# Tom-Ryder/VIforSDEs

Measured on AMD Instinct MI355X. Metric: sampled-paths/sec + ELBO-iters/sec (value = global_batch * ELBO-iters/s), higher is better.
Workload: dtype f32 (GRU/ELBO kernels) + bf16-autocast encoder

## Files before the change

include/vsde_hip.h:

```cpp
#ifndef VSDE_HIP_H
#define VSDE_HIP_H

#include <stddef.h>
#include <stdint.h>

#ifdef __cplusplus
extern "C" {
#endif

#define VSDE_ABI_VERSION 1

#define VSDE_E_BADARG (-1)
#define VSDE_E_LAYERS (-2)
#define VSDE_E_HIDDEN (-3)
#define VSDE_E_WORKSPACE (-4)
#define VSDE_E_STATE (-5)

#define VSDE_MAX_LAYERS 4
#define VSDE_MAX_HIDDEN 1024
#define VSDE_MAX_STATE 32

#define VSDE_CTX_F32 0
#define VSDE_CTX_BF16 1

// ... 59 lines not shown

int vsde_elbo_path_terms_bwd(int B, int T, int S, const float *z, const float *x,
                             const float *means, const float *chol, const float *drift,
                             const float *diffusion, const uint8_t *positive_mask_host,
                             double time_step, const float *g_sde, const float *g_gen,
                             const float *g_jac, float *g_z, float *g_x, float *g_means,
                             float *g_chol, float *g_drift, float *g_diffusion, void *stream);

int vsde_ln_modulate_fwd(int dtype, const void *x, const void *scale, const void *shift, void *y, float *mean,
                         float *rstd, int64_t B, int N, int C, double eps, int64_t mod_pitch, void *stream);
size_t vsde_colsum_workspace_bytes(int64_t B, int C);
int vsde_ln_modulate_bwd(int dtype, const void *x, const void *scale, const void *dy, const float *mean,
                         const float *rstd, const void *dres, void *dx, void *dscale, void *dshift, int64_t B, int N, int C,
                         int64_t mod_pitch, void *workspace, size_t workspace_bytes, void *stream);
int vsde_residual_ln_fwd(int dtype, const void *x, const void *y, const void *gate, const void *scale, const void *shift,
                         void *xnew, void *h, float *mean, float *rstd, int64_t B, int N, int C, double eps, int64_t mod_pitch,
                         void *stream);
int vsde_residual_ln_bwd(int dtype, const void *xnew, const void *y, const void *gate, const void *scale, const void *dh,
                         const void *dxnew, const float *mean, const float *rstd, void *dx, void *dy, void *dgate,
                         void *dscale, void *dshift, int64_t B, int N, int C, int64_t mod_pitch, void *workspace,
                         size_t workspace_bytes, void *stream);
int vsde_gated_residual_fwd(int dtype, const void *x, const void *y, const void *gate, void *out, int64_t B, int N, int C,
                            int64_t mod_pitch, void *stream);
int vsde_gated_residual_bwd(int dtype, const void *y, const void *gate, const void *dout, void *dy, void *dgate, int64_t B,
                            int N, int C, int64_t mod_pitch, void *workspace, size_t workspace_bytes, void *stream);
int vsde_swiglu_fwd(int dtype, const void *u, void *out, int64_t M, int H2, void *stream);
int vsde_swiglu_bwd(int dtype, const void *u, const void *dout, void *du, int64_t M, int H2, void *stream);
int vsde_gate_merge_fwd(int dtype, const void *attn, const void *glog, void *out, int64_t B, int N, int heads, int d,
                        int token_major, int64_t glog_stride, void *stream);
int vsde_gate_merge_bwd(int dtype, const void *attn, const void *glog, const void *dout, void *dattn, void *dglog, int64_t B,
                        int N, int heads, int d, int token_major, int64_t glog_stride, void *stream);
int vsde_qk_norm_rope_fwd(int dtype, const void *qkv, const float *cosT, const float *sinT, const float *wq, const float *wk,
                          const void *v0, const float *lam, void *q, void *k, void *v, int64_t B, int N, int heads, int d,
                          double eps, int token_major, int64_t row_stride, void *stream);
int64_t vsde_qk_norm_rope_bwd_partials(int64_t B, int N, int heads, int d);
int vsde_qk_norm_rope_bwd(int dtype, const void *qkv, const float *cosT, const float *sinT, const float *wq, const float *wk,
                          const void *v0, const float *lam, const void *dq, const void *dk, const void *dv, void *dqkv,
                          void *dv0, float *dlam_partial, int64_t B, int N, int heads, int d, double eps, int token_major,
                          int64_t row_stride, int dv0_accumulate, const void *dv_extra, void *stream);

int vsde_attention_max_tokens(void);
int vsde_attention_fwd_bf16(const void *q, const void *k, const void *v, void *o, float *lse, int64_t B, int N, int H,
                            int head_dim, double scale, void *stream);
int vsde_attention_bwd_bf16(const void *dout, const void *q, const void *k, const void *v, const void *o, const float *lse,
                            void *dq, void *dk, void *dv, float *delta, int64_t B, int N, int H, int head_dim, double scale,
                            void *stream);

int vsde_attention_fused_supported(int N, int head_dim);
int vsde_attention_fwd_gated_bf16(const void *q, const void *k, const void *v, const void *gate, int64_t ldg, void *o, float *lse,
                                  int64_t B, int N, int H, double scale, void *stream);
int vsde_gate_bwd_delta(const void *dout, const void *og, const void *gate, int64_t ldg, void *dattn, void *dgate, int64_t ldd,
                        float *delta, int64_t B, int N, int H, void *stream);
int64_t vsde_attention_bwd_fused_partials(int64_t B, int N, int H);
int vsde_attention_bwd_fused_bf16(const void *dattn, const void *q, const void *k, const void *v, const float *lse, const float *delta,
                                  const float *rinv, const float *cosT, const float *sinT, const float *wq, const float *wk,
                                  const void *vdiff, const float *lam, void *dv0, int dv0_accumulate, const void *dv_extra, void *dy,
                                  int64_t ldy, float *dlam_partial, int64_t B, int N, int H, double scale, void *stream);

size_t vsde_linear_wgrad_workspace_bytes(int64_t M, int N, int K);
int vsde_linear_wgrad_bf16(const void *dy, const void *x, int64_t M, int N, int K, float *dW, float *db, void *workspace,
                           size_t workspace_bytes, void *stream);
int vsde_linear_wgrad_bf16_rows(const void *dy, const void *x, int64_t M, int N, int K, float *dW, float *db,
                                const int32_t *row_map, void *workspace, size_t workspace_bytes, void *stream);
typedef struct VsdeWgradItem {
    const void *dy, *x;
    int64_t M;
    int32_t N, K;
    float *dW, *db;
    const int32_t *row_map;
} VsdeWgradItem;
size_t vsde_linear_wgrad_group_workspace_bytes(int n, const void *items );
int vsde_linear_wgrad_group_bf16(int n, const void *items, int group_plan, void *workspace, size_t workspace_bytes, void *stream);

#define VSDE_EPI_PLAIN 0
#define VSDE_EPI_SWIGLU 1
#define VSDE_EPI_SWIGLU_BWD 2
int vsde_linear_bf16_supported(int64_t M, int N, int K, int epilogue);
int vsde_linear_bf16(const void *x, int64_t ldx, const void *w, const void *bias, void *y, int64_t ldy, int64_t M, int N, int K,
                     int epilogue, void *s_out, int64_t lds, const void *u_in, int64_t ldu, void *stream);
int vsde_linear_qknorm_bf16(const void *x, int64_t ldx, const void *w, const void *bias, int64_t M, int K, int heads, int gate_width,
                            int tokens, const float *cosT, const float *sinT, const float *wq, const float *wk, const void *v0,
                            const float *lam, double eps, void *q, void *k, void *v, void *gate, int64_t ldg, int gate_sigmoid,
                            float *rinv, void *vdiff, void *stream);
int vsde_linear_gated_bf16(const void *attn, int64_t ldx, const void *gate, int64_t ldgate, const void *w, const void *bias, void *y,
                           int64_t ldy, int64_t M, int N, int K, void *stream);

int vsde_linear_gate_bwd_bf16(const void *dy, int64_t ldy, const void *w_t, const void *og, const void *s, int64_t lds, void *dattn,
                              void *dgate, int64_t ldd, float *delta, int64_t M, int K, int heads, int tokens, void *stream);

int vsde_mlp_block_fwd_bf16(const void *x, const void *yin, const void *ga, const void *sc, const void *sh, const void *gm,
                            const void *sn, const void *hs, int64_t mp, int tokens, double eps, double eps_next, const void *w1_img,
                            const void *w2_img, const float *b1_img, const void *b2, void *tok, void *hnext, int64_t M, int C, int H,
                            void *stream);
int vsde_mlp_attn_block_fwd_bf16(const void *x, const void *attn, const void *glog, int64_t ldg, const void *wo_img, const void *bo,
                                 const void *ga, const void *sc, const void *sh, const void *gm, const void *sn, const void *hs,
                                 int64_t mp, int tokens, double eps, double eps_next, const void *w1_img, const void *w2_img,
                                 const float *b1_img, const void *b2, void *tok, void *hnext, int64_t M, int C, int H, void *stream);
int vsde_linear_deep256_bf16(const void *x, int64_t ldx, const void *w_img, const void *bias, void *y, int64_t ldy, int64_t M, int K,
                             void *stream);
int64_t vsde_mlp_bwd_image_bytes(int C);
int vsde_mlp_bwd_bf16(const void *dy, int64_t lddy, const void *u, int64_t ldu, const void *img, void *du, int64_t lddu, void *dx,
                      int64_t lddx, int64_t M, int C, int H, void *stream);
int vsde_mlp_debug_trace(void *buf);
int vsde_wgrad_debug_trace(void *buf);
int vsde_attn_debug_trace(void *buf);
int vsde_mlp_image_bytes(int C, int64_t *w1_tile, int64_t *w2_tile, int64_t *b1_tile);
int vsde_mlp_fwd_bf16(const void *x, int64_t ldx, const void *w1_img, const void *w2_img, const float *b1_img, const void *b2, void *y,
                      int64_t ldy, void *s_out, int64_t lds, int64_t M, int C, int H, void *stream);

int vsde_optim_chunk_bytes(void);
int vsde_optim_chunk_elems(void);
int vsde_optim_step(const void *chunks, int n_chunks, const void *grads, const float *scale, float *partials, float *tstate,
                    const double *groups, double max_norm, double ema_weight, float *out, void *stream);

int vsde_pack_tile_bytes(void);
int vsde_pack_refresh(const void *tiles, int n_tiles, void *stream);

#define VSDE_SDE_OU 1
#define VSDE_SDE_LOTKA_VOLTERRA 2
#define VSDE_SDE_LINEAR_DIAGONAL 3
int vsde_euler_maruyama_fwd(int kind, int B, int T, int S, int P, const float *x0, const float *theta, const float *noise,
                            double time_step, const uint8_t *positive_mask_host, float *traj, void *stream);
int vsde_euler_maruyama_bwd(int kind, int B, int T, int S, int P, const float *theta, const float *noise, const float *traj,
                            const float *g_traj, double time_step, const uint8_t *positive_mask_host, float *g_x0,
                            float *g_theta, void *stream);

int vsde_elbo_tail_fwd(int B, int K, int S, int O, int P, const float *x_obs, const float *obs_values, const float *obs_matrix,
                       double variance, const float *theta, int prior_type, double prior_mean, double prior_std,
                       const float *post_mean, const float *post_log_std, const uint8_t *theta_positive_mask_host,
                       const float *sde_lp, const float *gen_lp, const float *log_jac, float *out6, void *stream);
int vsde_elbo_tail_bwd(int B, int K, int S, int O, int P, const float *x_obs, const float *obs_values, const float *obs_matrix,
                       double variance, const float *theta, int prior_type, double prior_mean, double prior_std,
                       const float *post_mean, const float *post_log_std, const uint8_t *theta_positive_mask_host,
                       const float *g_out6, float *g_x_obs, float *g_theta, float *g_post_mean, float *g_post_log_std,
                       float *g_sde, float *g_gen, float *g_jac, void *stream);

int vsde_sde_coefficients_fwd(int kind, int B, int T, int S, int P, const float *x, const float *theta, float *drift,
                              float *diffusion, void *stream);
int vsde_sde_coefficients_bwd(int kind, int B, int T, int S, int P, const float *x, const float *theta, const float *g_drift,
                              const float *g_diffusion, float *g_x, float *g_theta, void *stream);

int vsde_profile_enable(int on);
int vsde_debug_force_v1(int on);
int vsde_debug_head_mp(int mode);
int vsde_head_mfma_range_exceeded(int clear);
int vsde_profile_elapsed_ms(int which, float *ms);

#ifdef __cplusplus
}
#endif
#endif
```

viforsdes_amd/_hip.py:

```python
from __future__ import annotations

import ctypes
import os
from typing import Optional, Sequence

import torch

from .build import LIB_PATH

VSDE_ABI_VERSION = 1
MAX_LAYERS = 4
MAX_HIDDEN = 1024
MAX_STATE = 32
DIAG_MIN = 1e-2


class HipLibraryError(RuntimeError):
    pass


class _Dims(ctypes.Structure):
    _fields_ = [(n, ctypes.c_int) for n in ("B", "T", "S", "P", "C", "H", "L")]


class _Weights(ctypes.Structure):
    _fields_ = [(n, ctypes.c_void_p) for n in (
        "W_ih_l0", "W_hh_l0", "b_ih_l0", "b_hh_l0", "W_ih_stack", "W_hh_stack",
        "b_ih_stack", "b_hh_stack", "out_weight", "out_bias")]


class _CtxView(ctypes.Structure):
    _fields_ = [("base", ctypes.c_void_p), ("dtype", ctypes.c_int),
                ("batch_stride", ctypes.c_int64), ("step_stride", ctypes.c_int64)]


class _Grads(ctypes.Structure):
    _fields_ = [(n, ctypes.c_void_p) for n in (
        "x0", "context", "theta", "W_ih_l0", "W_hh_l0", "b_ih_l0", "b_hh_l0",
        "W_ih_stack", "W_hh_stack", "b_ih_stack", "b_hh_stack", "out_weight", "out_bias")] + [
        ("context_dtype", ctypes.c_int), ("context_batch_stride", ctypes.c_int64)]


EXPORTS = (
    "vsde_abi_version", "vsde_build_ablations", "vsde_last_error",
    "vsde_head_forward_workspace_bytes", "vsde_head_forward",
    "vsde_head_backward_workspace_bytes", "vsde_head_backward",
    "vsde_elbo_path_terms", "vsde_elbo_path_terms_bwd", "vsde_elbo_tail_fwd", "vsde_elbo_tail_bwd",
    "vsde_profile_enable", "vsde_profile_elapsed_ms", "vsde_debug_force_v1", "vsde_debug_head_mp", "vsde_head_mfma_range_exceeded",
    "vsde_ln_modulate_fwd", "vsde_ln_modulate_bwd", "vsde_gated_residual_fwd", "vsde_gated_residual_bwd",
    "vsde_swiglu_fwd", "vsde_swiglu_bwd", "vsde_gate_merge_fwd", "vsde_gate_merge_bwd",
    "vsde_qk_norm_rope_fwd", "vsde_qk_norm_rope_bwd_partials", "vsde_qk_norm_rope_bwd",
    "vsde_residual_ln_fwd", "vsde_residual_ln_bwd", "vsde_colsum_workspace_bytes", "vsde_linear_wgrad_workspace_bytes", "vsde_linear_wgrad_bf16", "vsde_linear_wgrad_bf16_rows", "vsde_linear_wgrad_group_workspace_bytes", "vsde_linear_wgrad_group_bf16",
    "vsde_attention_max_tokens", "vsde_attention_fwd_bf16", "vsde_attention_bwd_bf16",
    "vsde_attention_fused_supported", "vsde_attention_fwd_gated_bf16", "vsde_gate_bwd_delta", "vsde_attention_bwd_fused_partials",
    "vsde_attention_bwd_fused_bf16",
    "vsde_euler_maruyama_fwd", "vsde_euler_maruyama_bwd", "vsde_sde_coefficients_fwd", "vsde_sde_coefficients_bwd", "vsde_linear_bf16_supported", "vsde_linear_bf16", "vsde_linear_qknorm_bf16", "vsde_linear_gated_bf16", "vsde_linear_gate_bwd_bf16",
    "vsde_mlp_image_bytes", "vsde_mlp_fwd_bf16", "vsde_mlp_block_fwd_bf16", "vsde_mlp_attn_block_fwd_bf16", "vsde_linear_deep256_bf16", "vsde_mlp_debug_trace", "vsde_wgrad_debug_trace", "vsde_attn_debug_trace", "vsde_mlp_bwd_image_bytes", "vsde_mlp_bwd_bf16",
    "vsde_pack_tile_bytes", "vsde_pack_refresh", "vsde_optim_chunk_bytes", "vsde_optim_chunk_elems", "vsde_optim_step",
)

_lib: Optional[ctypes.CDLL] = None
_loaded_path: Optional[str] = None


def library_path() -> str:
    return _loaded_path or os.environ.get("VSDE_HIP_LIB") or LIB_PATH


def has_ablations() -> bool:
    return bool(load().vsde_build_ablations())


ABL_LIB_PATH = os.path.join(os.path.dirname(LIB_PATH), "libvsde_hip_abl.so")


def load() -> ctypes.CDLL:
    global _lib
    if _lib is not None:
        return _lib
    path = os.environ.get("VSDE_HIP_LIB") or LIB_PATH
    if not os.path.exists(path):
        raise HipLibraryError(
            f"{path} is missing: build it with `python -m viforsdes_amd.build` "
            "(there is no CPU fallback for the fused head / ELBO kernels)")
    lib = ctypes.CDLL(path)
    for name in EXPORTS:
        if not hasattr(lib, name):
            raise HipLibraryError(f"{path} does not export {name}")
    global _loaded_path
    _loaded_path = path
    lib.vsde_abi_version.restype = ctypes.c_int
    if lib.vsde_abi_version() != VSDE_ABI_VERSION:
        raise HipLibraryError(f"{path}: ABI version mismatch; rebuild it")
    lib.vsde_last_error.restype = ctypes.c_char_p
    lib.vsde_head_forward_workspace_bytes.restype = ctypes.c_size_t
    lib.vsde_head_backward_workspace_bytes.restype = ctypes.c_size_t
    for f in (lib.vsde_head_forward, lib.vsde_head_backward, lib.vsde_elbo_path_terms, lib.vsde_elbo_path_terms_bwd):
        f.restype = ctypes.c_int
    lib.vsde_qk_norm_rope_bwd_partials.restype = ctypes.c_int64
    lib.vsde_attention_bwd_fused_partials.restype = ctypes.c_int64
    lib.vsde_linear_wgrad_workspace_bytes.restype = ctypes.c_size_t
    lib.vsde_linear_wgrad_group_workspace_bytes.restype = ctypes.c_size_t
    lib.vsde_colsum_workspace_bytes.restype = ctypes.c_size_t
    lib.vsde_mlp_bwd_image_bytes.restype = ctypes.c_int64
    _lib = lib
    return lib


def _raise(rc: int) -> None:
    msg = load().vsde_last_error().decode("utf-8", "replace")
    if rc < 0:
        raise ValueError(msg)
    raise HipLibraryError(f"HIP error {rc}: {msg}")


def _ptr(t: Optional[torch.Tensor]):
    return ctypes.c_void_p(None if t is None or t.numel() == 0 else t.data_ptr())


def _require_hip(*tensors: torch.Tensor) -> torch.device:
    dev = None
    for t in tensors:
        if t is None:
            continue
        if not t.is_cuda:
            raise HipLibraryError(
                "the fused head / ELBO kernels only run on a HIP (cuda) device; got a "
                f"{t.device} tensor and there is no CPU fallback")
        if dev is None:
            dev = t.device
        elif t.device != dev:
            raise ValueError("all tensors must live on the same device")
    assert dev is not None
    return dev


def _stream(dev: torch.device):
    return ctypes.c_void_p(torch.cuda.current_stream(dev).cuda_stream)

# ... 562 lines not shown
    n = len(problems)
    items = (_WgradItem * n)()
    outs = []
    for i, (dy, x, want_bias, row_map, out_rows) in enumerate(problems):
        M, N = dy.shape
        K = x.shape[1]
        rows = N if row_map is None else int(out_rows)
        dW = torch.empty(rows, K, device=dev, dtype=torch.float32)
        db = torch.empty(rows, device=dev, dtype=torch.float32) if want_bias else None
        items[i] = _WgradItem(dy.data_ptr(), x.data_ptr(), M, N, K, dW.data_ptr(), None if db is None else db.data_ptr(),
                              None if row_map is None else row_map.data_ptr())
        outs.append((dW, db))
    nbytes = lib.vsde_linear_wgrad_group_workspace_bytes(ctypes.c_int(n), ctypes.byref(items))
    ws = torch.empty(nbytes, device=dev, dtype=torch.uint8)
    with torch.cuda.device(dev):
        _call(lib.vsde_linear_wgrad_group_bf16, ctypes.c_int(n), ctypes.byref(items), ctypes.c_int(1 if group_plan else 0), _ptr(ws),
              ctypes.c_size_t(nbytes), _stream(dev))
    return outs


EPI_PLAIN, EPI_SWIGLU, EPI_SWIGLU_BWD = 0, 1, 2


def linear_variant(M: int, N: int, K: int, epilogue: int = EPI_PLAIN) -> int:
    return int(load().vsde_linear_bf16_supported(_i64(M), ctypes.c_int(N), ctypes.c_int(K), ctypes.c_int(epilogue)))


def linear_supported(M: int, N: int, K: int, epilogue: int = EPI_PLAIN) -> bool:
    return linear_variant(M, N, K, epilogue) != 0


def _rows2d(t: torch.Tensor):
    if t.dtype != torch.bfloat16 or t.ndim != 2 or t.stride(1) != 1:
        raise ValueError(f"expected a row-pitched bf16 matrix, got {t.dtype} {tuple(t.shape)} strides {t.stride()}")
    return t, t.stride(0)


def linear_bf16(x: torch.Tensor, w: torch.Tensor, bias: Optional[torch.Tensor], out: Optional[torch.Tensor] = None):
    lib = load(); dev = _require_hip(x, w)
    x, ldx = _rows2d(x)
    M, K = x.shape
    N = w.shape[0]
    y = torch.empty(M, N, device=dev, dtype=torch.bfloat16) if out is None else out
    with torch.cuda.device(dev):
        _call(lib.vsde_linear_bf16, _ptr(x), _i64(ldx), _ptr(w), _ptr(bias), _ptr(y), _i64(y.stride(0)), _i64(M), ctypes.c_int(N),
              ctypes.c_int(K), ctypes.c_int(EPI_PLAIN), None, _i64(0), None, _i64(0), _stream(dev))
    return y


def linear_swiglu_bf16(x: torch.Tensor, w: torch.Tensor, bias: Optional[torch.Tensor], want_u: bool = True):
    lib = load(); dev = _require_hip(x, w)
    x, ldx = _rows2d(x)
    M, K = x.shape
    N = w.shape[0]
    u = torch.empty(M, N, device=dev, dtype=torch.bfloat16) if want_u else None
    s = torch.empty(M, N // 2, device=dev, dtype=torch.bfloat16)
    with torch.cuda.device(dev):
        _call(lib.vsde_linear_bf16, _ptr(x), _i64(ldx), _ptr(w), _ptr(bias), _ptr(u), _i64(N), _i64(M), ctypes.c_int(N),
              ctypes.c_int(K), ctypes.c_int(EPI_SWIGLU), _ptr(s), _i64(N // 2), None, _i64(0), _stream(dev))
    return u, s


def linear_qknorm_bf16(x: torch.Tensor, w: torch.Tensor, bias: Optional[torch.Tensor], heads: int, tokens: int, cos, sin, wq, wk,
                       v0: Optional[torch.Tensor], lam: Optional[torch.Tensor], eps: float, save: bool = False):
    lib = load(); dev = _require_hip(x, w, cos, sin, wq, wk)
    x, ldx = _rows2d(x)
    M, K = x.shape
    C = heads * 64
    G = w.shape[0] - 3 * C
    q = torch.empty(M, C, device=dev, dtype=torch.bfloat16); k = torch.empty_like(q); v = torch.empty_like(q)
    gate = torch.empty(M, G, device=dev, dtype=torch.bfloat16) if G > 0 else None
    rinv = torch.empty(M, 2 * heads, device=dev, dtype=torch.float32) if save else None
    vdiff = torch.empty(M, C, device=dev, dtype=torch.bfloat16) if (save and v0 is not None) else None
    with torch.cuda.device(dev):
        _call(lib.vsde_linear_qknorm_bf16, _ptr(x), _i64(ldx), _ptr(w), _ptr(bias), _i64(M), ctypes.c_int(K), ctypes.c_int(heads),
              ctypes.c_int(G), ctypes.c_int(tokens), _ptr(cos), _ptr(sin), _ptr(wq), _ptr(wk), _ptr(v0), _ptr(lam),
              ctypes.c_double(eps), _ptr(q), _ptr(k), _ptr(v), _ptr(gate), _i64(G), ctypes.c_int(int(save)), _ptr(rinv), _ptr(vdiff),
              _stream(dev))
    if save:
        return q, k, v, gate, rinv, vdiff
    return q, k, v, gate


def attention_fused_supported(N: int, head_dim: int) -> bool:
    return bool(load().vsde_attention_fused_supported(ctypes.c_int(N), ctypes.c_int(head_dim)))


def attention_fwd_gated(q: torch.Tensor, k: torch.Tensor, v: torch.Tensor, gate: torch.Tensor, scale: float):
    lib = load(); dev = _require_hip(q, k, v, gate)
    B, N, H, d = q.shape
    if q.dtype != torch.bfloat16 or d != 64 or not (q.is_contiguous() and k.is_contiguous() and v.is_contiguous()):
        raise ValueError("attention_fwd_gated needs contiguous bf16 [B,N,H,64] tensors")
    gate, ldg = _rows2d(gate)
    o = torch.empty_like(q)
    lse = torch.empty(B, H, N, device=dev, dtype=torch.float32)
    with torch.cuda.device(dev):
        _call(lib.vsde_attention_fwd_gated_bf16, _ptr(q), _ptr(k), _ptr(v), _ptr(gate), _i64(ldg), _ptr(o), _ptr(lse), _i64(B),
              ctypes.c_int(N), ctypes.c_int(H), ctypes.c_double(scale), _stream(dev))
    return o, lse


def gate_bwd_delta(dout: torch.Tensor, og: torch.Tensor, gate: torch.Tensor, dgate: torch.Tensor):
    lib = load(); dev = _require_hip(dout, og, gate, dgate)
    B, N, H, d = og.shape
    if d != 64 or not (dout.is_contiguous() and og.is_contiguous()) or dout.dtype != torch.bfloat16:
        raise ValueError("gate_bwd_delta needs contiguous bf16 [B,N,H,64] tensors")
    gate, ldg = _rows2d(gate); dgate, ldd = _rows2d(dgate)
    dattn = torch.empty_like(og)
    delta = torch.empty(B, H, N, device=dev, dtype=torch.float32)
    with torch.cuda.device(dev):
        _call(lib.vsde_gate_bwd_delta, _ptr(dout), _ptr(og), _ptr(gate), _i64(ldg), _ptr(dattn), _ptr(dgate), _i64(ldd), _ptr(delta),
              _i64(B), ctypes.c_int(N), ctypes.c_int(H), _stream(dev))
    return dattn, delta


def mlp_image_bytes(C: int) -> tuple[int, int, int]:
    a, b, c = ctypes.c_int64(0), ctypes.c_int64(0), ctypes.c_int64(0)
    rc = load().vsde_mlp_image_bytes(ctypes.c_int(C), ctypes.byref(a), ctypes.byref(b), ctypes.byref(c))
    if rc != 0:
        _raise(rc)
    return int(a.value), int(b.value), int(c.value)


def mlp_fwd(x: torch.Tensor, w1_img: torch.Tensor, w2_img: torch.Tensor, b1_img: torch.Tensor, b2: Optional[torch.Tensor], H: int,
            want_s: bool = False):
    lib = load(); dev = _require_hip(x, w1_img, w2_img, b1_img)
    x, ldx = _rows2d(x)
    M, C = x.shape
    y = torch.empty(M, C, device=dev, dtype=torch.bfloat16)
    s = torch.empty(M, H, device=dev, dtype=torch.bfloat16) if want_s else None
    with torch.cuda.device(dev):
        _call(lib.vsde_mlp_fwd_bf16, _ptr(x), _i64(ldx), _ptr(w1_img), _ptr(w2_img), _ptr(b1_img), _ptr(b2), _ptr(y), _i64(C), _ptr(s),
              _i64(H), _i64(M), ctypes.c_int(C), ctypes.c_int(H), _stream(dev))
    return y, s


def mlp_block_fwd(x, yin, ga, sc, sh, gm, sn, hs, eps: float, eps_next: float, w1_img, w2_img, b1_img, b2, H: int):
    lib = load(); dev = _require_hip(x, yin, ga, sc, sh, gm, w1_img, w2_img, b1_img)
    B, N, C = x.shape
    if not (x.is_contiguous() and yin.is_contiguous() and x.dtype == torch.bfloat16 and yin.dtype == torch.bfloat16 and yin.shape == x.shape):
        raise ValueError("mlp_block_fwd: x and yin must be contiguous bf16 tensors of one shape")
    mp = _mod_pitch(C, ga, sc, sh, gm, sn, hs)
    tok = torch.empty_like(x)
    hnext = torch.empty_like(x) if sn is not None else None
    with torch.cuda.device(dev):
        _call(lib.vsde_mlp_block_fwd_bf16, _ptr(x), _ptr(yin), _ptr(ga), _ptr(sc), _ptr(sh), _ptr(gm), _ptr(sn), _ptr(hs), _i64(mp),
              ctypes.c_int(N), ctypes.c_double(eps), ctypes.c_double(eps_next), _ptr(w1_img), _ptr(w2_img), _ptr(b1_img), _ptr(b2),
              _ptr(tok), _ptr(hnext), _i64(B * N), ctypes.c_int(C), ctypes.c_int(H), _stream(dev))
    return tok, hnext


def mlp_attn_block_fwd(x, attn, glog, wo_img, bo, ga, sc, sh, gm, sn, hs, eps: float, eps_next: float, w1_img, w2_img, b1_img, b2, H: int):
    lib = load(); dev = _require_hip(x, attn, glog, wo_img, ga, sc, sh, gm, w1_img, w2_img, b1_img)
    B, N, C = x.shape
    if not (x.is_contiguous() and attn.is_contiguous() and x.dtype == torch.bfloat16 and attn.dtype == torch.bfloat16 and attn.numel() == x.numel()):
        raise ValueError("mlp_attn_block_fwd: x and attn must be contiguous bf16 tensors of one size")
    if not (glog.ndim == 2 and glog.shape == (B * N, 64) and glog.dtype == torch.bfloat16 and glog.stride(1) == 1):
        raise ValueError("mlp_attn_block_fwd: glog must be [B*N, 64] bf16 with unit column stride")
    mp = _mod_pitch(C, ga, sc, sh, gm, sn, hs)
    tok = torch.empty_like(x)
    hnext = torch.empty_like(x) if sn is not None else None
    with torch.cuda.device(dev):
        _call(lib.vsde_mlp_attn_block_fwd_bf16, _ptr(x), _ptr(attn), _ptr(glog), _i64(glog.stride(0)), _ptr(wo_img), _ptr(bo), _ptr(ga), _ptr(sc),
              _ptr(sh), _ptr(gm), _ptr(sn), _ptr(hs), _i64(mp), ctypes.c_int(N), ctypes.c_double(eps), ctypes.c_double(eps_next), _ptr(w1_img),
              _ptr(w2_img), _ptr(b1_img), _ptr(b2), _ptr(tok), _ptr(hnext), _i64(B * N), ctypes.c_int(C), ctypes.c_int(H), _stream(dev))
    return tok, hnext
# ... 86 lines not shown
```

viforsdes_amd/csrc/vsde_common.h:

```cpp
#pragma once
#include <hip/hip_runtime.h>
#include <stdint.h>
#include <stdio.h>
#include <stdlib.h>

#include "../../include/vsde_hip.h"

namespace vsde {

constexpr int kWave = 64;
constexpr int kHP = 64;
constexpr int kChunks = 16;
constexpr int kMatF4 = kChunks * 3 * kHP;

void set_error(const char *fmt, ...);

#ifdef VSDE_ABLATIONS
static inline long long vsde_knob(const char *name, long long dflt) {
    const char *e = getenv(name);
    return (e && *e) ? atoll(e) : dflt;
}
static inline int ablation_env(const char *name) {
    const char *e = getenv(name);
    const int v = e ? atoi(e) : 0;
    if (v != 0) fprintf(stderr, "libvsde_hip: %s=%d is a TIMING-ONLY ablation switch -- results of the affected kernels are WRONG\n", name, v);
    return v;
}
#else
#define vsde_knob(name, dflt) ((long long)(dflt))
#define ablation_env(name) (0)
#endif

#define VSDE_CHECK_ARG(cond, code, ...)          \
    do {                                         \
        if (!(cond)) {                           \
            vsde::set_error(__VA_ARGS__);        \
            return (code);                       \
        }                                        \
    } while (0)

#define VSDE_CHECK_HIP(expr)                                                         \
    do {                                                                             \
        hipError_t e_ = (expr);                                                      \
        if (e_ != hipSuccess) {                                                      \
            vsde::set_error("%s failed: %s", #expr, hipGetErrorString(e_));          \
            return (int)e_;                                                          \
        }                                                                            \
    } while (0)

struct RowView {
    const void *base;
    int64_t batch_stride;
    int64_t row_stride;
    int rows_per_batch;
    int shift;
    int col_split;
    int col_skip;
    int dtype;
};

__device__ __forceinline__ float bf16_to_f32(uint16_t v) { return __uint_as_float(((uint32_t)v) << 16); }

__device__ __forceinline__ int64_t rowview_offset(const RowView &v, int m, bool &valid) {
    int b = m / v.rows_per_batch;
    int t = m - b * v.rows_per_batch + v.shift;
    valid = t >= 0;
    return (int64_t)b * v.batch_stride + (int64_t)t * v.row_stride;
}

__device__ __forceinline__ float rowview_load(const RowView &v, int64_t off, int k) {
    int kk = k < v.col_split ? k : k + v.col_skip;
    if (v.dtype == 0) return ((const float *)v.base)[off + kk];
    return bf16_to_f32(((const uint16_t *)v.base)[off + kk]);
}

__device__ __forceinline__ float fast_rcp(float x) { return __builtin_amdgcn_rcpf(x); }
__device__ __forceinline__ float fast_exp2(float x) { return __builtin_amdgcn_exp2f(x); }
__device__ __forceinline__ float fast_sigmoid(float x) { return fast_rcp(1.0f + fast_exp2(-1.4426950408889634f * x)); }
__device__ __forceinline__ float fast_tanh(float x) { return 1.0f - 2.0f * fast_rcp(1.0f + fast_exp2(2.8853900817779268f * x)); }

__device__ __forceinline__ void wave_lds_fence() {
    __builtin_amdgcn_fence(__ATOMIC_RELEASE, "wavefront");
    __builtin_amdgcn_wave_barrier();
    __builtin_amdgcn_fence(__ATOMIC_ACQUIRE, "wavefront");
}

__device__ __forceinline__ float sum_xor32(float v) {
    const uint32_t u = __float_as_uint(v);
    const auto s = __builtin_amdgcn_permlane32_swap(u, u, false, false);
    return __uint_as_float(s[0]) + __uint_as_float(s[1]);
}

__device__ __forceinline__ float xor32(float v) {
    const uint32_t u = __float_as_uint(v);
    const auto s = __builtin_amdgcn_permlane32_swap(u, u, false, false);
    return __uint_as_float((threadIdx.x & 32) ? s[0] : s[1]);
}
template <int K>
__device__ __forceinline__ float xor_lane(float v) {
    static_assert(K > 0 && K < 32, "ds_swizzle bit mode reaches the 32 lanes of a half wave");
    return __int_as_float(__builtin_amdgcn_ds_swizzle(__float_as_int(v), (K << 10) | 0x1f));
}

__device__ __forceinline__ float wave_sum(float v) {
#pragma unroll
    for (int off = 32; off > 0; off >>= 1) v += __shfl_xor(v, off, 64);
    return v;
}

__device__ __forceinline__ void transpose8x8(const uint4 (&r)[8], uint4 (&c)[8]) {
    const uint32_t *rr = (const uint32_t *)r;
    uint32_t *cc = (uint32_t *)c;
#pragma unroll
    for (int j = 0; j < 8; ++j)
#pragma unroll
        for (int p = 0; p < 4; ++p) {
            const uint32_t a = rr[(2 * p) * 4 + (j >> 1)], b = rr[(2 * p + 1) * 4 + (j >> 1)];
            cc[j * 4 + p] = (j & 1) ? __builtin_amdgcn_perm(b, a, 0x07060302u) : __builtin_amdgcn_perm(b, a, 0x05040100u);
        }
}

template <int CTRL> __device__ __forceinline__ float dpp_add(float v) {
    return v + __int_as_float(__builtin_amdgcn_update_dpp(0, __float_as_int(v), CTRL, 0xf, 0xf, true));
}

__device__ __forceinline__ float wave_sum_of_quads(float v) {
    v = dpp_add<0x141>(v);
    v = dpp_add<0x140>(v);
    const float r0 = __int_as_float(__builtin_amdgcn_readlane(__float_as_int(v), 0));
    const float r1 = __int_as_float(__builtin_amdgcn_readlane(__float_as_int(v), 16));
    const float r2 = __int_as_float(__builtin_amdgcn_readlane(__float_as_int(v), 32));
    const float r3 = __int_as_float(__builtin_amdgcn_readlane(__float_as_int(v), 48));
    return (r0 + r1) + (r2 + r3);
}

int launch_gemm_nt(const RowView &A, int M, int K, const float *Bt, int ldb, int N, const float *bias,
                   float *C, int64_t ldc, hipStream_t stream, int out_rpb = 0, int64_t out_bstride = 0, int out_dtype = 0);

struct TnProblem {
    RowView X;
    RowView Y;
    int NX, NY;
    float *out;
    int64_t ldo;
    int col_off;
    float *bias_out;
};
constexpr int kMaxTnProblems = 12;
size_t tn_workspace_bytes(const TnProblem *probs, int nprob, int M);
int launch_tn_grouped(const TnProblem *probs, int nprob, int M, void *workspace, size_t workspace_bytes,
                      hipStream_t stream);

size_t tn_wide_workspace_bytes(const TnProblem *probs, int nprob, int M);
int launch_tn_wide(const TnProblem *probs, int nprob, int M, void *workspace, size_t workspace_bytes, hipStream_t stream);

size_t proj_planes_bytes(int N, int K);
int launch_proj_fwd_bf16(const RowView &A, int64_t M, int K, const float *W, int ldw, int N, const float *bias, float *G, int64_t ldc,
                         void *scratch, size_t scratch_bytes, hipStream_t s);
int launch_proj_bwd_bf16(const RowView &A, int64_t M, int K, const float *Wt, int ldw, int N, void *C, int64_t ldc, int out_rpb,
                         int64_t out_bstride, void *scratch, size_t scratch_bytes, hipStream_t s);

struct MpLaunch {
    int B, T, S, P, C, L, save;
    int np;
    const float *x0, *theta, *eps, *G;
    const float *W_ih0, *W_hh0, *W_ih_st, *W_hh_st, *out_W;
    const float *b_hh0, *b_ih_st, *b_hh_st, *out_b;
    void *frags;
    float dt, sqdt, diag_min;
    float *paths, *means, *chol, *chol_raw, *acts;
};
bool mp_applicable(int H, int L, int S);
bool mp_weights_overflowed();
void mp_clear_overflow();
size_t mp_frag_bytes(int L, int S);
int launch_head_fwd_mp(const MpLaunch &a, hipStream_t s, void (*mark)(int, int, hipStream_t));

struct MpBwdLaunch {
    int B, T, S, P, C;
    int np;
    const float *g_paths, *g_means, *g_chol, *eps, *chol_raw, *acts;
    const float *W_ih0, *W_hh0, *W_ih_st, *W_hh_st, *out_W;
    void *frags;
    float dt, sqdt, diag_min;
// ... 13 lines not shown
```

viforsdes_amd/csrc/vsde_encoder.hip:

```cpp
#include <stdlib.h>

#include "vsde_common.h"

namespace vsde {

struct bf16_t { uint16_t v; };

__device__ __forceinline__ float to_f32(float x) { return x; }
__device__ __forceinline__ float to_f32(bf16_t x) { return __uint_as_float(((uint32_t)x.v) << 16); }
template <typename T> __device__ __forceinline__ T from_f32(float x);
template <> __device__ __forceinline__ float from_f32<float>(float x) { return x; }
template <> __device__ __forceinline__ bf16_t from_f32<bf16_t>(float x) {
    uint32_t u = __float_as_uint(x);
    if ((u & 0x7fffffffu) > 0x7f800000u) return bf16_t{(uint16_t)((u >> 16) | 0x40)};
    u += 0x7fffu + ((u >> 16) & 1u);
    return bf16_t{(uint16_t)(u >> 16)};
}
template <typename T> __device__ __forceinline__ float rnd(float x) { return to_f32(from_f32<T>(x)); }

__device__ __forceinline__ float sigm(float x) { return fast_rcp(1.0f + __expf(-x)); }

template <typename T, int V> struct Pack;
template <int V> struct Pack<float, V> {
    static __device__ __forceinline__ void load(const float *p, float (&o)[V]) {
// ... 1 lines not shown
        else if (V == 2) { float2 t = *(const float2 *)p; o[0] = t.x; o[1] = t.y; }
        else {
#pragma unroll
            for (int i = 0; i < V; ++i) o[i] = p[i];
        }
    }
    static __device__ __forceinline__ void store(float *p, const float (&o)[V]) {
        if (V == 4) *(float4 *)p = make_float4(o[0], o[1], o[2], o[3]);
        else if (V == 2) *(float2 *)p = make_float2(o[0], o[1]);
        else {
#pragma unroll
            for (int i = 0; i < V; ++i) p[i] = o[i];
        }
    }
};
template <int V> struct Pack<bf16_t, V> {
    static __device__ __forceinline__ void load(const bf16_t *p, float (&o)[V]) {
        if (V == 8) { uint4 t = *(const uint4 *)p; const uint32_t w[4] = {t.x, t.y, t.z, t.w};
#pragma unroll
            for (int i = 0; i < 4; ++i) { o[2 * i] = __uint_as_float(w[i] << 16); o[2 * i + 1] = __uint_as_float(w[i] & 0xffff0000u); } }
        else if (V == 4) { uint2 t = *(const uint2 *)p; const uint32_t w[2] = {t.x, t.y};
#pragma unroll
            for (int i = 0; i < 2; ++i) { o[2 * i] = __uint_as_float(w[i] << 16); o[2 * i + 1] = __uint_as_float(w[i] & 0xffff0000u); } }
        else if (V == 2) { uint32_t w = *(const uint32_t *)p; o[0] = __uint_as_float(w << 16); o[1] = __uint_as_float(w & 0xffff0000u); }
        else {
#pragma unroll
            for (int i = 0; i < V; ++i) o[i] = to_f32(p[i]);
        }
    }
    static __device__ __forceinline__ void store(bf16_t *p, const float (&o)[V]) {
        if (V == 8 || V == 4 || V == 2) {
            uint32_t w[V / 2 > 0 ? V / 2 : 1];
#pragma unroll
            for (int i = 0; i < V / 2; ++i) w[i] = (uint32_t)from_f32<bf16_t>(o[2 * i]).v | ((uint32_t)from_f32<bf16_t>(o[2 * i + 1]).v << 16);
            if (V == 8) *(uint4 *)p = make_uint4(w[0], w[1], w[2 % (V / 2)], w[3 % (V / 2)]);
            else if (V == 4) *(uint2 *)p = make_uint2(w[0], w[1 % (V / 2)]);
            else *(uint32_t *)p = w[0];
        } else {
#pragma unroll
            for (int i = 0; i < V; ++i) p[i] = from_f32<bf16_t>(o[i]);
        }
    }
};
template <typename T> struct VecOf { static constexpr int v = 4; };
template <> struct VecOf<bf16_t> { static constexpr int v = 8; };

__device__ __forceinline__ float seg_sum(float v, int width) {
    for (int off = width >> 1; off > 0; off >>= 1) v += __shfl_xor(v, off, 64);
    return v;
}

template <typename T, int V, int LPR, int NSLAB>
__global__ void __launch_bounds__(256) ln_mod_fwd_kernel(const T *__restrict__ x, const T *__restrict__ scale,
                                                         const T *__restrict__ shift, T *__restrict__ y,
                                                         float *__restrict__ mean, float *__restrict__ rstd, int64_t M,
                                                         int N, int C, float eps, const T *__restrict__ res_y,
                                                         const T *__restrict__ res_gate, T *__restrict__ xnew, int64_t mp) {
    const int lane = threadIdx.x & (LPR - 1);
    constexpr int nslab = NSLAB;
    const int64_t stride = (int64_t)gridDim.x * (256 / LPR);
    int64_t m = (int64_t)blockIdx.x * (256 / LPR) + threadIdx.x / LPR;
    float v[NSLAB][V], ry[NSLAB][V], nv[NSLAB][V], nry[NSLAB][V];
    auto fetch = [&](int64_t mm, float (&vx)[NSLAB][V], float (&vy)[NSLAB][V]) {
#pragma unroll
        for (int sl = 0; sl < NSLAB; ++sl)
            if (sl < nslab) {
                Pack<T, V>::load(x + mm * C + (sl * LPR + lane) * V, vx[sl]);
                if (res_y) Pack<T, V>::load(res_y + mm * C + (sl * LPR + lane) * V, vy[sl]);
            }
    };
    if (m < M) fetch(m, v, ry);
    for (; m < M; m += stride) {
        const int64_t mn = m + stride;
        if (mn < M) fetch(mn, nv, nry);
        const int64_t b = m / N;
        float s = 0.f;
#pragma unroll
        for (int sl = 0; sl < NSLAB; ++sl)
            if (sl < nslab) {
                if (res_y) {
                    float rg[V];
                    Pack<T, V>::load(res_gate + b * mp + (sl * LPR + lane) * V, rg);
#pragma unroll
                    for (int e = 0; e < V; ++e) v[sl][e] = rnd<T>(v[sl][e] + rnd<T>(rg[e] * ry[sl][e]));
                    Pack<T, V>::store(xnew + m * C + (sl * LPR + lane) * V, v[sl]);
                }
#pragma unroll
                for (int e = 0; e < V; ++e) s += v[sl][e];
            }
        const float mu = seg_sum(s, LPR) / C;
        float q = 0.f;
#pragma unroll
        for (int sl = 0; sl < NSLAB; ++sl)
            if (sl < nslab)
#pragma unroll
                for (int e = 0; e < V; ++e) { const float d = v[sl][e] - mu; q += d * d; }
        const float rs = rsqrtf(seg_sum(q, LPR) / C + eps);
        if (lane == 0) { mean[m] = mu; rstd[m] = rs; }
#pragma unroll
        for (int sl = 0; sl < NSLAB; ++sl)
            if (sl < nslab) {
                const int c = (sl * LPR + lane) * V;
                float sc[V], sh[V], o[V];
                Pack<T, V>::load(scale + b * mp + c, sc); Pack<T, V>::load(shift + b * mp + c, sh);
#pragma unroll
                for (int e = 0; e < V; ++e) o[e] = (v[sl][e] - mu) * rs * (1.0f + sc[e]) + sh[e];
                Pack<T, V>::store(y + m * C + c, o);
            }
#pragma unroll
        for (int sl = 0; sl < NSLAB; ++sl)
#pragma unroll
            for (int e = 0; e < V; ++e) { v[sl][e] = nv[sl][e]; ry[sl][e] = nry[sl][e]; }
    }
}

constexpr int kColsumChunksMax = 64;
static int colsum_chunks(int64_t B, int N) {
    static int force = -1;
    if (force < 0) force = (int)vsde_knob("VSDE_COLSUM_CHUNKS", 0);
    if (force > 0) return force > kColsumChunksMax ? kColsumChunksMax : (force > N ? (N > 0 ? N : 1) : force);
    int64_t c = (768 + B - 1) / B;
    if (c < 4) c = 4;
    if (c > kColsumChunksMax) c = kColsumChunksMax;
    if (c > N / 8) c = N / 8 > 0 ? N / 8 : 1;
    return (int)c;
}

template <int NACC>
__device__ __forceinline__ void colsum_block_reduce(float *red, const float (&acc)[NACC], int slot, int slots, int lane_off,
                                                    int width, float *__restrict__ part, int C) {
    __syncthreads();
#pragma unroll
    for (int e = 0; e < NACC; ++e) red[slot * width + lane_off + e] = acc[e];
    __syncthreads();
    for (int c = threadIdx.x; c < width && c < C; c += blockDim.x) {
        float t = 0.f;
        for (int sidx = 0; sidx < slots; ++sidx) t += red[sidx * width + c];
        part[c] = t;
    }
}

template <typename T, int V, int LPR, int NSLAB>
__global__ void __launch_bounds__(256) ln_mod_bwd_kernel(const T *__restrict__ x, const T *__restrict__ scale,
                                                         const T *__restrict__ dy, const float *__restrict__ mean,
                                                         const float *__restrict__ rstd, const T *__restrict__ dres,
                                                         T *__restrict__ dx, float *__restrict__ part, int N, int C,
                                                         const T *__restrict__ res_y, const T *__restrict__ res_gate,
                                                         T *__restrict__ res_dy, int64_t mp) {
    extern __shared__ float red[];
    constexpr int SLOTS = 256 / LPR;
    const int lane = threadIdx.x & (LPR - 1), slot = threadIdx.x / LPR;
    const int b = blockIdx.y, nchunk = gridDim.x, B = gridDim.y;
    const int CL = (N + nchunk - 1) / nchunk;
    const int n0 = blockIdx.x * CL, n1 = min(N, n0 + CL);
    constexpr int nslab = NSLAB;
    float sc1[NSLAB][V], a1[NSLAB][V], a2[NSLAB][V], a3[NSLAB][V], gt[NSLAB][V];
#pragma unroll
    for (int sl = 0; sl < NSLAB; ++sl) {
        if (sl < nslab) {
            Pack<T, V>::load(scale + (int64_t)b * mp + (sl * LPR + lane) * V, sc1[sl]);
#pragma unroll
            for (int e = 0; e < V; ++e) sc1[sl][e] += 1.0f;
            if (res_y) Pack<T, V>::load(res_gate + (int64_t)b * mp + (sl * LPR + lane) * V, gt[sl]);
        }
#pragma unroll
        for (int e = 0; e < V; ++e) { a1[sl][e] = 0.f; a2[sl][e] = 0.f; a3[sl][e] = 0.f; }
    }
    for (int n = n0 + slot; n < n1; n += SLOTS) {
        const int64_t m = (int64_t)b * N + n;
        const float mu = mean[m], rs = rstd[m];
        float g[NSLAB][V], xh[NSLAB][V];
        float s1 = 0.f, s2 = 0.f;
#pragma unroll
        for (int sl = 0; sl < NSLAB; ++sl)
            if (sl < nslab) {
                const int c = (sl * LPR + lane) * V;
                Pack<T, V>::load(x + m * C + c, xh[sl]); Pack<T, V>::load(dy + m * C + c, g[sl]);
#pragma unroll
                for (int e = 0; e < V; ++e) {
                    xh[sl][e] = (xh[sl][e] - mu) * rs;
                    a1[sl][e] += g[sl][e] * xh[sl][e]; a2[sl][e] += g[sl][e];
                    g[sl][e] *= sc1[sl][e];
                    s1 += g[sl][e]; s2 += g[sl][e] * xh[sl][e];
                }
            }
        s1 = seg_sum(s1, LPR) / C; s2 = seg_sum(s2, LPR) / C;
#pragma unroll
        for (int sl = 0; sl < NSLAB; ++sl)
            if (sl < nslab) {
// ... 656 lines not shown
```

viforsdes_amd/csrc/vsde_linear.hip:

```cpp
#include <stdlib.h>

#include "vsde_common.h"

namespace vsde {

typedef float f32x16 __attribute__((ext_vector_type(16)));
typedef short bf16x8 __attribute__((ext_vector_type(8)));
typedef uint32_t u32x4 __attribute__((ext_vector_type(4)));

constexpr int EPI_PLAIN = 0, EPI_SWIGLU = 1, EPI_SWIGLU_BWD = 2, EPI_QKNORM = 3, EPI_GATE_BWD = 4;
constexpr int R2_THREADS = 256, R2_SLD = 88;

struct LinParams {
    const uint16_t *A; int64_t lda;
    const uint16_t *W;
    const uint16_t *bias;
    uint16_t *C; int64_t ldc;
    uint16_t *S; int64_t lds_;
    const uint16_t *U; int64_t ldu;
    int64_t M; int N, K;
    int chunks;
    int tail_local, tail_chunks;
    uint16_t *Qo, *Ko, *Vo, *Go; int64_t ldg;
    const float *cosT, *sinT, *wq, *wk, *lam;
    const uint16_t *V0;
    int heads, tokens; float eps;
    int gate_sigmoid;
    const uint16_t *Og; const uint16_t *Sg; int64_t ldsg;
    uint16_t *Dgate; int64_t lddg;
    float *Delta;
    float *Rinv;
    uint16_t *Vdiff;
    const uint16_t *Gate; int64_t ldgate;
    int dbg;
    int xstage;
};

typedef __bf16 hwbf16x2 __attribute__((ext_vector_type(2)));
typedef float f32x2 __attribute__((ext_vector_type(2)));
__device__ __forceinline__ uint32_t pack_bf16x2(float lo, float hi) {
    const f32x2 v = {lo, hi};
    return __builtin_bit_cast(uint32_t, __builtin_convertvector(v, hwbf16x2));
}
__device__ __forceinline__ float bf_lo(uint32_t w) { return __uint_as_float(w << 16); }
__device__ __forceinline__ float bf_hi(uint32_t w) { return __uint_as_float(w & 0xffff0000u); }
__device__ __forceinline__ float rbf(float x) { return (float)(__bf16)x; }
__device__ __forceinline__ void lds_barrier() { asm volatile("s_waitcnt lgkmcnt(0)\n\ts_barrier" ::: "memory"); }

__device__ __forceinline__ float sigm_f(float x) { return fast_rcp(1.0f + __expf(-x)); }

template <int SLD, int R>
__device__ __forceinline__ void flush_rows64(const uint16_t *stage, uint16_t *dst, int64_t ld, int64_t row0, int64_t M, int lane) {
#pragma unroll
    for (int i = 0; i < R / 8; ++i) {
        const int row = (lane >> 3) + 8 * i, c = lane & 7;
        const u32x4 v = *(const u32x4 *)(stage + row * SLD + c * 8);
        if (row0 + row < M) __builtin_nontemporal_store(v, (u32x4 *)(dst + (row0 + row) * ld + c * 8));
    }
}
template <int SLD, int R>
__device__ __forceinline__ void flush_rows32(const uint16_t *stage, uint16_t *dst, int64_t ld, int64_t row0, int64_t M, int lane) {
#pragma unroll
    for (int i = 0; i < R / 16; ++i) {
        const int row = (lane >> 2) + 16 * i, c = lane & 3;
        const u32x4 v = *(const u32x4 *)(stage + row * SLD + c * 8);
        if (row0 + row < M) __builtin_nontemporal_store(v, (u32x4 *)(dst + (row0 + row) * ld + c * 8));
    }
}

__device__ __forceinline__ void stage_block(const f32x16 &acc, const uint16_t *bias32, uint16_t *dst_row, int h) {
    uint2 bb[4];
#pragma unroll
    for (int g = 0; g < 4; ++g) bb[g] = *(const uint2 *)(bias32 + 8 * g + 4 * h);
#pragma unroll
    for (int g = 0; g < 4; ++g)
        *(uint2 *)(dst_row + 8 * g + 4 * h) = make_uint2(pack_bf16x2(acc[4 * g + 0] + bf_lo(bb[g].x), acc[4 * g + 1] + bf_hi(bb[g].x)),
                                                        pack_bf16x2(acc[4 * g + 2] + bf_lo(bb[g].y), acc[4 * g + 3] + bf_hi(bb[g].y)));
}

template <int NLD, int KW, int THREADS>
__device__ __forceinline__ void wtile_load(u32x4 (&breg)[NLD], const uint16_t *W, int64_t ldw, int tid) {
#pragma unroll
    for (int i = 0; i < NLD; ++i) {
        const int idx = tid + THREADS * i, row = idx / (KW / 8), c = idx % (KW / 8);
        breg[i] = *(const u32x4 *)(W + (int64_t)row * ldw + c * 8);
    }
}
template <int NLD, int KW, int LDB, int THREADS>
__device__ __forceinline__ void wtile_store(const u32x4 (&breg)[NLD], uint16_t *Bs, int tid) {
#pragma unroll
    for (int i = 0; i < NLD; ++i) {
        const int idx = tid + THREADS * i, row = idx / (KW / 8), c = idx % (KW / 8);
        *(u32x4 *)(Bs + row * LDB + c * 8) = breg[i];
    }
}

__device__ __forceinline__ void swiglu_quads(const f32x16 &acc, const uint16_t *bias32, int h, uint32_t (&out)[4]) {
#pragma unroll
    for (int g = 0; g < 2; ++g) {
        const uint2 ba = *(const uint2 *)(bias32 + 8 * g + 4 * h), bb = *(const uint2 *)(bias32 + 16 + 8 * g + 4 * h);
        const float av[4] = {bf_lo(ba.x), bf_hi(ba.x), bf_lo(ba.y), bf_hi(ba.y)};
        const float bv[4] = {bf_lo(bb.x), bf_hi(bb.x), bf_lo(bb.y), bf_hi(bb.y)};
        float sv[4];
#pragma unroll
        for (int i = 0; i < 4; ++i) {
            const float a = rbf(acc[4 * g + i] + av[i]), b = rbf(acc[4 * (g + 2) + i] + bv[i]);
            sv[i] = rbf(a * sigm_f(a)) * b;
        }
        out[2 * g] = pack_bf16x2(sv[0], sv[1]); out[2 * g + 1] = pack_bf16x2(sv[2], sv[3]);
    }
}

__device__ __forceinline__ void swiglu_stage(const f32x16 &acc, const uint16_t *bias32, uint16_t *dst_row, int h, uint32_t (&out)[4]) {
    uint32_t uw[4][2];
    uint2 bbv[4];
#pragma unroll
    for (int g = 0; g < 4; ++g) bbv[g] = *(const uint2 *)(bias32 + 8 * g + 4 * h);
#pragma unroll
// ... 177 lines not shown
                for (int rb = 0; rb < RB; ++rb) {
#pragma unroll
                    for (int g = 0; g < 2; ++g) *(uint2 *)(stage + (rb * 32 + r) * SLD + 8 * g + 4 * h) = make_uint2(sq[rb][2 * g], sq[rb][2 * g + 1]);
                }
                wave_lds_fence();
#pragma unroll
                for (int i = 0; i < R / 16; ++i) {
                    const int row = (lane >> 2) + 16 * i, c = lane & 3;
                    const u32x4 v = *(const u32x4 *)(stage + row * SLD + (c < 2 ? 64 + 8 * c : 8 * (c - 2)));
                    if (row0 + row < p.M) __builtin_nontemporal_store(v, (u32x4 *)(p.S + (row0 + row) * p.lds_ + ((n0 - 32) >> 1) + c * 8));
                }
            }
            wave_lds_fence();
        }
    } else {
#pragma unroll
        for (int i = 0; i < 4 * RB; ++i) {
            const int row = (lane >> 3) + 8 * i, c = lane & 7;
            *(u32x4 *)(stage + row * SLD + c * 8) = ureg[i];
        }
        wave_lds_fence();
#pragma unroll
        for (int rb = 0; rb < RB; ++rb) {
            uint2 uav[4], ubv[4];
#pragma unroll
            for (int g = 0; g < 4; ++g) {
                const uint16_t *pa = stage + (rb * 32 + r) * SLD + 32 * (g >> 1) + 8 * (g & 1) + 4 * h;
                uav[g] = *(const uint2 *)pa; ubv[g] = *(const uint2 *)(pa + 16);
            }
#pragma unroll
            for (int g = 0; g < 4; ++g) {
                uint16_t *pa = stage + (rb * 32 + r) * SLD + 32 * (g >> 1) + 8 * (g & 1) + 4 * h, *pb = pa + 16;
                const uint2 ua = uav[g], ub = ubv[g];
                const float a[4] = {bf_lo(ua.x), bf_hi(ua.x), bf_lo(ua.y), bf_hi(ua.y)};
                const float b[4] = {bf_lo(ub.x), bf_hi(ub.x), bf_lo(ub.y), bf_hi(ub.y)};
                float da[4], db[4];
#pragma unroll
                for (int i = 0; i < 4; ++i) {
                    const float gs = acc[rb][4 * g + i], sg = sigm_f(a[i]);
                    da[i] = gs * b[i] * sg * (1.0f + a[i] * (1.0f - sg));
                    db[i] = gs * a[i] * sg;
                }
                *(uint2 *)pa = make_uint2(pack_bf16x2(da[0], da[1]), pack_bf16x2(da[2], da[3]));
                *(uint2 *)pb = make_uint2(pack_bf16x2(db[0], db[1]), pack_bf16x2(db[2], db[3]));
            }
        }
        wave_lds_fence();
        flush_rows64<SLD, R>(stage, p.C + 2 * n0, p.ldc, row0, p.M, lane);
        wave_lds_fence();
    }
}

template <int EPI, int NKH = 1> constexpr int rows_rb() { return (EPI == EPI_SWIGLU_BWD || EPI == EPI_QKNORM || EPI == EPI_GATE_BWD || NKH > 1) ? 1 : 2; }

template <int KC, int RB, int KSTOT, int K0, bool ZERO>
__device__ __forceinline__ void rows_tile_mfma(f32x16 (&acc)[RB], const bf16x8 (&afr)[RB][KSTOT], const uint16_t *bsrc) {
    constexpr int KS = KC / 16, GK = RB == 1 ? 4 : 2, NG = KS / GK;
    if constexpr (ZERO) {
#pragma unroll
        for (int rb = 0; rb < RB; ++rb)
#pragma unroll
            for (int e = 0; e < 16; ++e) acc[rb][e] = 0.f;
    }
    bf16x8 bq[2][GK];
#pragma unroll
    for (int k = 0; k < GK; ++k) bq[0][k] = *(const bf16x8 *)(bsrc + k * 16);
    __builtin_amdgcn_s_setprio(1);
#pragma unroll
    for (int gk = 0; gk < NG; ++gk) {
        if (gk + 1 < NG)
#pragma unroll
            for (int k = 0; k < GK; ++k) bq[(gk + 1) & 1][k] = *(const bf16x8 *)(bsrc + ((gk + 1) * GK + k) * 16);
        __builtin_amdgcn_sched_barrier(0);
#pragma unroll
        for (int k = 0; k < GK; ++k)
#pragma unroll
            for (int rb = 0; rb < RB; ++rb)
                acc[rb] = __builtin_amdgcn_mfma_f32_32x32x16_bf16(bq[gk & 1][k], afr[rb][K0 + gk * GK + k], acc[rb], 0, 0, 0);
        __builtin_amdgcn_sched_barrier(0);
    }
    __builtin_amdgcn_s_setprio(0);
}

template <int KC, int EPI, int NKH, int NW>
__global__ void __launch_bounds__(64 * NW, NW == 4 ? 2 : 1) lin_rows_kernel(LinParams p) {
    constexpr int RB = rows_rb<EPI, NKH>(), ROWS = 32 * NW * RB, THREADS = 64 * NW;
    constexpr int KS = NKH * KC / 16, KT = NKH * KC, LDB = KC + 8, TILE = 33 * LDB;
    constexpr int NLD = 32 * KC / 8 / THREADS;
    extern __shared__ __attribute__((aligned(16))) uint16_t lsm[];
    const int tid = threadIdx.x, lane = tid & 63, wave = tid >> 6, r = lane & 31, h = lane >> 5;
    uint16_t *stage = lsm + 2 * TILE + wave * (32 * RB * R2_SLD);
    const int xcd = blockIdx.x & 7, local = blockIdx.x >> 3;
    const bool tail = local >= p.tail_local;
    const int nchunks = tail ? p.tail_chunks : p.chunks, lrel = tail ? local - p.tail_local : local;
    const int chunk = lrel % nchunks;
    const int64_t stripe = (int64_t)(lrel / nchunks + (tail ? p.tail_local / p.chunks : 0)) * 8 + xcd;
    if (stripe * ROWS >= p.M) return;
    const int64_t row0 = stripe * ROWS + wave * (32 * RB);

    bf16x8 afr[RB][KS];
    const bool xst = NKH == 1 && p.xstage && !(EPI == EPI_PLAIN && p.Gate != nullptr);
    if (xst) {
        constexpr int CPR = KT / 8, RPI = 64 / CPR;
        char *xs = (char *)lsm + wave * (32 * KT * 2);
        const int lrow = lane / CPR, lc = lane % CPR;
#pragma unroll
        for (int rb = 0; rb < RB; ++rb) {
            u32x4 t[KS];
#pragma unroll
            for (int i = 0; i < KS; ++i) {
                const int rl = i * RPI + lrow;
                const int64_t m = row0 + rb * 32 + rl < p.M ? row0 + rb * 32 + rl : p.M - 1;
                t[i] = *(const u32x4 *)(p.A + m * p.lda + lc * 8);
            }
            if (rb > 0) wave_lds_fence();
#pragma unroll
            for (int i = 0; i < KS; ++i) {
                const int rl = i * RPI + lrow;
                *(u32x4 *)(xs + rl * (KT * 2) + ((lc ^ (rl & 15)) << 4)) = t[i];
            }
            wave_lds_fence();
#pragma unroll
            for (int ks = 0; ks < KS; ++ks) afr[rb][ks] = *(const bf16x8 *)(xs + r * (KT * 2) + (((h + 2 * ks) ^ (r & 15)) << 4));
        }
        lds_barrier();
    }
#pragma unroll
    for (int rb = 0; rb < RB; ++rb) {
        if (xst) break;
        const int64_t m = row0 + rb * 32 + r < p.M ? row0 + rb * 32 + r : p.M - 1;
        const uint16_t *src = p.A + m * p.lda + 8 * h;
#pragma unroll
        for (int ks = 0; ks < KS; ++ks) afr[rb][ks] = *(const bf16x8 *)(src + ks * 16);
        if (EPI == EPI_PLAIN && NKH == 1 && p.Gate != nullptr) {
            const uint16_t *gsrc = p.Gate + m * p.ldgate + 8 * h;
#pragma unroll
            for (int ks = 0; ks < KS; ++ks) {
                const u32x4 a = __builtin_bit_cast(u32x4, afr[rb][ks]), g = *(const u32x4 *)(gsrc + (ks & 3) * 16);
                u32x4 o;
#pragma unroll
                for (int e = 0; e < 4; ++e)
                    o[e] = pack_bf16x2(bf_lo(a[e]) * rbf(sigm_f(bf_lo(g[e]))), bf_hi(a[e]) * rbf(sigm_f(bf_hi(g[e]))));
                afr[rb][ks] = __builtin_bit_cast(bf16x8, o);
            }
        }
    }
    __shared__ float wlds[128];
    if constexpr (EPI == EPI_QKNORM) { if (tid < 128) wlds[tid] = tid < 64 ? p.wq[tid] : p.wk[tid - 64]; }
    float cs[16], sn[16];
#pragma unroll
    for (int e = 0; e < 16; ++e) { cs[e] = EPI == EPI_GATE_BWD ? 0.f : 1.f; sn[e] = 0.f; }
    if constexpr (EPI == EPI_QKNORM) {
        const int64_t m = row0 + r < p.M ? row0 + r : p.M - 1;
        const int64_t tok = m % p.tokens;
#pragma unroll
        for (int q = 0; q < 4; ++q) {
            const float4 c4 = *(const float4 *)(p.cosT + tok * 32 + 16 * h + 4 * q), s4 = *(const float4 *)(p.sinT + tok * 32 + 16 * h + 4 * q);
            cs[4 * q] = c4.x; cs[4 * q + 1] = c4.y; cs[4 * q + 2] = c4.z; cs[4 * q + 3] = c4.w;
            sn[4 * q] = s4.x; sn[4 * q + 1] = s4.y; sn[4 * q + 2] = s4.z; sn[4 * q + 3] = s4.w;
        }
    }
    const int pairs_all = p.N / 64, ppc = (pairs_all + nchunks - 1) / nchunks, pair0 = chunk * ppc;
    const int ntiles = 2 * (ppc < pairs_all - pair0 ? ppc : pairs_all - pair0), tile0 = 2 * pair0;
    if (ntiles <= 0) return;
    const int rot = 2 * ((int)stripe % (ntiles / 2));
    u32x4 breg[NLD];
    uint32_t biasreg = 0u;
    u32x4 ureg[4 * RB];
#define VSDE_TILE_LOAD(q_)                                                                                    \
    do {                                                                                                      \
        const int tile_ = tile0 + ((q_) / NKH + rot) % ntiles;                                                \
        wtile_load<NLD, KC, THREADS>(breg, p.W + (int64_t)tile_ * 32 * KT + ((q_) % NKH) * KC, KT, tid);      \
        if (tid < 16) biasreg = p.bias ? *(const uint32_t *)(p.bias + tile_ * 32 + 2 * (lane_t & 15)) : 0u;   \
    } while (0)
#define VSDE_TILE_STORE(Bs_)                                                                                  \
    do {                                                                                                      \
        wtile_store<NLD, KC, LDB, THREADS>(breg, (Bs_), tid);                                                 \
        if (tid < 16) *(uint32_t *)((Bs_) + 32 * LDB + 2 * tid) = biasreg;                                    \
    } while (0)
#define VSDE_U_LOAD(t_)                                                                                       \
    do {                                                                                                      \
        if constexpr (EPI == EPI_QKNORM) {    \
            const int tl_ = tile0 + ((t_) + rot) % ntiles, pp_ = tl_ >> 1, kind_ = pp_ / p.heads;              \
            if (p.V0 != nullptr && (tl_ & 1) == 0 && kind_ == 2) {                                            \
                const int64_t m_ = row0 + (lane_t & 31) < p.M ? row0 + (lane_t & 31) : p.M - 1;               \
                const uint16_t *v_ = p.V0 + m_ * ((int64_t)p.heads * 64) + (pp_ - 2 * p.heads) * 64 + 16 * (lane_t >> 5); \
                ureg[0] = *(const u32x4 *)v_; ureg[1] = *(const u32x4 *)(v_ + 8);                             \
                ureg[2] = *(const u32x4 *)(v_ + 32); ureg[3] = *(const u32x4 *)(v_ + 40);                     \
            }                                                                                                 \
        }                                                                                                     \
        if constexpr (EPI == EPI_GATE_BWD) {    \
            const int tl_ = tile0 + ((t_) + rot) % ntiles;                                                    \
            if ((tl_ & 1) == 0) {                                                                             \
                _Pragma("unroll") for (int i = 0; i < 4; ++i) {                                               \
                    const int row = (lane_t >> 3) + 8 * i, c = lane_t & 7;                                    \
                    const int64_t m_ = row0 + row < p.M ? row0 + row : p.M - 1;                               \
                    ureg[i] = *(const u32x4 *)(p.Og + m_ * (int64_t)p.N + (tl_ >> 1) * 64 + c * 8);           \
                }                                                                                             \
            }                                                                                                 \
        }                                                                                                     \
        if constexpr (EPI == EPI_SWIGLU_BWD) {                                                                \
            const int n0_ = (tile0 + ((t_) + rot) % ntiles) * 32;                                             \
            _Pragma("unroll") for (int i = 0; i < 4 * RB; ++i) {                                              \
                const int row = (lane >> 3) + 8 * i, c = lane & 7;                                            \
                const int64_t m_ = row0 + row < p.M ? row0 + row : p.M - 1;                                   \
                ureg[i] = *(const u32x4 *)(p.U + m_ * p.ldu + 2 * n0_ + c * 8);                               \
// ... 183 lines not shown
                asm volatile("s_barrier" ::: "memory");
                if (wave < 4) { if (kt + 2 < nk) issue(kt + 2); }
                else if (kt + 1 < nk) issue(kt + 1);
                if (active && p.dbg < 5) {
                    const uint32_t sa = (uint32_t)(uintptr_t)(dlds + (kt % DP_ASTAGES) * DP_HALF + a_base);
                    const uint32_t sw = (uint32_t)(uintptr_t)(dlds + (kt % DP_WSTAGES) * DP_HALF + w_base);
                    bf16x8 fa[2][2], fw[2][4];
#define VSDE_FRAG(dst_, addr_, off_) asm volatile("ds_read_b128 %0, %1 offset:%2" : "=v"(dst_) : "v"(addr_), "i"(off_))
#define VSDE_FRAGS(par_, ks_)                                                                                  \
                    do {                                                                                       \
                        const uint32_t a_ = sa + fo[ks_], w_ = sw + fo[ks_];                                   \
                        VSDE_FRAG(fa[par_][0], a_, 0); VSDE_FRAG(fw[par_][0], w_, 0); VSDE_FRAG(fw[par_][1], w_, 4096);   \
                        VSDE_FRAG(fa[par_][1], a_, 4096); VSDE_FRAG(fw[par_][2], w_, 8192); VSDE_FRAG(fw[par_][3], w_, 12288); \
                    } while (0)
#define VSDE_MFMAS(par_)                                                                                       \
                    do {                                                                                       \
                        _Pragma("unroll") for (int nb = 0; nb < 4; ++nb)                                       \
                            _Pragma("unroll") for (int rb = 0; rb < 2; ++rb)                                   \
                                acc[rb][nb] = __builtin_amdgcn_mfma_f32_32x32x16_bf16(fw[par_][nb], fa[par_][rb], acc[rb][nb], 0, 0, 0); \
                    } while (0)
                    VSDE_FRAGS(0, 0);
                    VSDE_FRAGS(1, 1);
                    __builtin_amdgcn_s_setprio(1);
                    asm volatile("s_waitcnt lgkmcnt(6)" ::: "memory");
                    __builtin_amdgcn_sched_barrier(0);
                    VSDE_MFMAS(0);
                    __builtin_amdgcn_sched_barrier(0);
                    VSDE_FRAGS(0, 2);
                    asm volatile("s_waitcnt lgkmcnt(6)" ::: "memory");
                    __builtin_amdgcn_sched_barrier(0);
                    VSDE_MFMAS(1);
                    __builtin_amdgcn_sched_barrier(0);
                    VSDE_FRAGS(1, 3);
                    asm volatile("s_waitcnt lgkmcnt(6)" ::: "memory");
                    __builtin_amdgcn_sched_barrier(0);
                    VSDE_MFMAS(0);
                    __builtin_amdgcn_sched_barrier(0);
                    asm volatile("s_waitcnt lgkmcnt(0)" ::: "memory");
                    __builtin_amdgcn_sched_barrier(0);
                    VSDE_MFMAS(1);
                    __builtin_amdgcn_s_setprio(0);
#undef VSDE_MFMAS
#undef VSDE_FRAGS
#undef VSDE_FRAG
                }
            }
            asm volatile("s_waitcnt lgkmcnt(0)\n\ts_barrier" ::: "memory");
            uint16_t *brow = (uint16_t *)dlds;
            uint16_t *stg = (uint16_t *)dlds + 256 + wave * (32 * DP_SLD);
            if (tid < 128) *(uint32_t *)(brow + 2 * tid) = p.bias ? *(const uint32_t *)(p.bias + ct * 256 + 2 * tid) : 0u;
            lds_barrier();
            if (active) {
#pragma unroll
                for (int rb = 0; rb < 2; ++rb)
#pragma unroll
                    for (int pr = 0; pr < 2; ++pr) {
                        const int n0 = wn * 128 + pr * 64;
                        stage_block(acc[rb][2 * pr], brow + n0, stg + r * DP_SLD, h);
                        stage_block(acc[rb][2 * pr + 1], brow + n0 + 32, stg + r * DP_SLD + 32, h);
                        wave_lds_fence();
                        flush_rows64<DP_SLD, 32>(stg, p.C + ct * 256 + n0, p.ldc, trow + wm * 64 + rb * 32, bound, lane);
                        wave_lds_fence();
                    }
            }
            lds_barrier();
        }
    }
}
#endif

static int rows_xstage() {
    static int v = -1;
    if (v < 0) v = (int)vsde_knob("VSDE_ROWS_XSTAGE", 1);
    return v;
}

template <int KC, int EPI, int NKH, int NW> static size_t rows_lds_bytes() {
    const size_t need = (size_t)(2 * 33 * (KC + 8) + NW * 32 * rows_rb<EPI, NKH>() * R2_SLD) * sizeof(uint16_t);
    const size_t xstage = NKH == 1 ? (size_t)NW * 32 * KC * 2 : 0;
    return need > xstage ? need : xstage;
}
template <int NB> static size_t cols_lds_bytes() { return (size_t)(2 * 32 * NB * C2_LDB) * sizeof(uint16_t); }

template <int KC, int EPI, int NKH, int NW>
static int launch_rows_nw(const LinParams &p, hipStream_t s) {
    const size_t lds = rows_lds_bytes<KC, EPI, NKH, NW>();
    VSDE_CHECK_HIP(hipFuncSetAttribute((const void *)lin_rows_kernel<KC, EPI, NKH, NW>, hipFuncAttributeMaxDynamicSharedMemorySize, (int)lds));
    constexpr int rows = 32 * NW * rows_rb<EPI, NKH>();
    constexpr int resident = NW == 4 ? 512 : 256;
    const int64_t stripes = (p.M + rows - 1) / rows;
    const int pairs = p.N / 64;
    int chunks = 1;
    if ((EPI == EPI_SWIGLU || EPI == EPI_SWIGLU_BWD || EPI == EPI_QKNORM) && stripes < resident && pairs >= 2) {
        int64_t c = (resident + stripes - 1) / stripes;
        if (c > pairs) c = pairs;
        const int64_t ppc = (pairs + c - 1) / c;
        chunks = (int)((pairs + ppc - 1) / ppc);
    } else {
        while (stripes * chunks < resident && chunks * 2 <= pairs && pairs % (chunks * 2) == 0) chunks *= 2;
    }
    {
        static int big = -1;
        if (big < 0) big = (int)vsde_knob("VSDE_ROWS_CHUNKS", 0);
        const bool uneven_ok = EPI == EPI_SWIGLU || EPI == EPI_SWIGLU_BWD;
        int want = big > 0 ? big : (EPI == EPI_PLAIN ? 1 : 2);
        if (big <= 0 && uneven_ok) {
            double best = 0.0;
            for (int c = 2; c <= 4; ++c) {
                if (pairs < 2 * c) break;
                const double rounds = (double)stripes * c / resident, eff = rounds / (double)(int64_t)(rounds + 0.999999) - 0.05 * c;
                if (eff > best) { best = eff; want = c; }
            }
        }
        if (stripes >= resident && want > 1 && (pairs % want == 0 || (uneven_ok && pairs >= 2 * want))) chunks = want;
    }
    if (EPI == EPI_GATE_BWD) chunks = 1;
    LinParams q = p;
    q.chunks = chunks;
    q.xstage = rows_xstage();
    const int64_t groups = (stripes + 7) / 8, wg_main = groups * 8 * chunks;
    int64_t tail_groups = 0; int tail_chunks = chunks;
    {
        static int on = -1;
        if (on < 0) on = (int)vsde_knob("VSDE_ROWS_TAIL", 1);
        const int64_t full = wg_main / resident * resident, rest = wg_main - full;
        const bool can_chunk = EPI != EPI_GATE_BWD && (EPI == EPI_SWIGLU || EPI == EPI_SWIGLU_BWD || EPI == EPI_QKNORM || EPI == EPI_PLAIN);
        if (on && can_chunk && full > 0 && rest >= 8 * (int64_t)chunks && rest * 2 <= resident) {
            const int64_t tg = (rest / chunks + 7) / 8;
            int tc = (int)(resident / (tg * 8));
            if (tc > pairs) tc = pairs;
            const bool even_only = EPI == EPI_PLAIN;
            while (tc > chunks && even_only && pairs % tc != 0) --tc;
            if (tc > chunks) { tail_groups = tg; tail_chunks = tc; }
        }
    }
    q.tail_local = (int)((groups - tail_groups) * chunks);
    q.tail_chunks = tail_chunks;
    const int64_t nwg = ((groups - tail_groups) * chunks + tail_groups * tail_chunks) * 8;
    hipLaunchKernelGGL((lin_rows_kernel<KC, EPI, NKH, NW>), dim3((unsigned)nwg), dim3(64 * NW), lds, s, q);
    VSDE_CHECK_HIP(hipGetLastError());
    return 0;
}

static int rows_wide_wg() {
    static int v = -1;
    if (v < 0) v = (int)vsde_knob("VSDE_ROWS_NW", 8);
    return v;
}
template <int KC, int EPI, int NKH = 1>
static int launch_rows(const LinParams &p, hipStream_t s) {
    if constexpr (NKH > 1 && EPI != EPI_QKNORM) {
        if (rows_wide_wg() == 8 && p.M >= 256 * 256) return launch_rows_nw<KC, EPI, NKH, 8>(p, s);
    }
    return launch_rows_nw<KC, EPI, NKH, 4>(p, s);
}

template <int EPI>
static int launch_rows_k(const LinParams &p, hipStream_t s) {
    if (p.K == 512) return launch_rows<256, EPI, 2>(p, s);
    return p.K == 128 ? launch_rows<128, EPI>(p, s) : launch_rows<256, EPI>(p, s);
}

template <int NB>
static int launch_cols(const LinParams &p, hipStream_t s) {
    const size_t lds = cols_lds_bytes<NB>();
    VSDE_CHECK_HIP(hipFuncSetAttribute((const void *)lin_cols_kernel<NB>, hipFuncAttributeMaxDynamicSharedMemorySize, (int)lds));
    const int64_t stripes = (p.M + C2_ROWS - 1) / C2_ROWS;
    hipLaunchKernelGGL((lin_cols_kernel<NB>), dim3((unsigned)(stripes * (p.N / (32 * NB)))), dim3(C2_THREADS), lds, s, p);
    VSDE_CHECK_HIP(hipGetLastError());
    return 0;
}

#ifdef VSDE_ABLATIONS
static int launch_deep(const LinParams &p, hipStream_t s) {
    static int cus = 0;
    if (!cus) {
        int dev = 0; hipDeviceProp_t prop;
        VSDE_CHECK_HIP(hipGetDevice(&dev));
        VSDE_CHECK_HIP(hipGetDeviceProperties(&prop, dev));
        cus = prop.multiProcessorCount > 0 ? prop.multiProcessorCount : 256;
    }
    const size_t lds = (size_t)DP_LDS_BYTES;
    VSDE_CHECK_HIP(hipFuncSetAttribute((const void *)lin_deep_kernel, hipFuncAttributeMaxDynamicSharedMemorySize, (int)lds));
    int64_t rows = (p.M + cus - 1) / cus;
    rows = (rows + 31) / 32 * 32;
    if (rows < 64) rows = 64;
    const int64_t wgs = (p.M + rows - 1) / rows;
    hipLaunchKernelGGL(lin_deep_kernel, dim3((unsigned)wgs), dim3(DP_THREADS), lds, s, p, (int)rows);
    VSDE_CHECK_HIP(hipGetLastError());
    return 0;
}
#endif

static int launch_qknorm(const LinParams &p, hipStream_t s) {
    return p.K == 128 ? launch_rows<128, EPI_QKNORM>(p, s) : launch_rows<256, EPI_QKNORM>(p, s);
}

#ifdef VSDE_ABLATIONS
static bool deep_enabled() {
    static int v = -1;
    if (v < 0) v = (int)vsde_knob("VSDE_DEEP_GEMM", 0);
    return v != 0;
}
#endif

static int lin_variant(int64_t M, int N, int K, int epilogue) {
#ifdef VSDE_ABLATIONS
    if (epilogue == EPI_PLAIN && deep_enabled() && K >= 512 && K % 64 == 0 && N % 256 == 0 && N <= K && M >= 32768) return 3;
#endif
    const bool rows_ok = (K == 128 || K == 256 || K == 512) && N % 64 == 0;
    const bool cols_ok = K % 64 == 0 && N % 128 == 0 && epilogue == EPI_PLAIN;
    if (epilogue != EPI_PLAIN) return rows_ok ? 1 : 0;
    if (rows_ok && (!cols_ok || N >= K)) return 1;
    return cols_ok ? 2 : (rows_ok ? 1 : 0);
}

}

using namespace vsde;

extern "C" int vsde_linear_bf16_supported(int64_t M, int N, int K, int epilogue) {
    if (M <= 0 || N <= 0 || K <= 0 || epilogue < 0 || epilogue > 2) return 0;
    return lin_variant(M, N, K, epilogue);
}

extern "C" int vsde_linear_bf16(const void *x, int64_t ldx, const void *w, const void *bias, void *y, int64_t ldy, int64_t M, int N,
                                int K, int epilogue, void *s_out, int64_t lds, const void *u_in, int64_t ldu, void *stream) {
    VSDE_CHECK_ARG(x && w && M > 0 && N > 0 && K > 0, VSDE_E_BADARG, "bad linear arguments");
    VSDE_CHECK_ARG(epilogue >= 0 && epilogue <= 2, VSDE_E_BADARG, "unknown linear epilogue %d", epilogue);
    const int variant = lin_variant(M, N, K, epilogue);
    VSDE_CHECK_ARG(variant != 0, VSDE_E_BADARG, "linear shape N=%d K=%d epilogue=%d is not covered by the gfx950 kernels", N, K, epilogue);
    VSDE_CHECK_ARG(ldx >= K && ldx % 8 == 0 && ((uintptr_t)x % 16) == 0 && ((uintptr_t)w % 16) == 0, VSDE_E_BADARG,
                   "linear operands must be 16-byte aligned with row pitches that are multiples of 8 elements");
    LinParams p = {};
    p.A = (const uint16_t *)x; p.lda = ldx; p.W = (const uint16_t *)w; p.bias = (const uint16_t *)bias;
    p.C = (uint16_t *)y; p.ldc = ldy; p.M = M; p.N = N; p.K = K;
    p.S = (uint16_t *)s_out; p.lds_ = lds; p.U = (const uint16_t *)u_in; p.ldu = ldu;
    { static int dbg = -1; if (dbg < 0) dbg = ablation_env("VSDE_LIN_DEBUG"); p.dbg = dbg; }
    hipStream_t st = (hipStream_t)stream;
    if (epilogue == EPI_PLAIN) {
        VSDE_CHECK_ARG(y && ldy >= N && ldy % 8 == 0 && ((uintptr_t)y % 16) == 0, VSDE_E_BADARG, "bad linear output");
        if (variant == 1) return launch_rows_k<EPI_PLAIN>(p, st);
#ifdef VSDE_ABLATIONS
        if (variant == 3) return launch_deep(p, st);
#endif
        return N % 256 == 0 ? launch_cols<8>(p, st) : launch_cols<4>(p, st);
    }
    if (epilogue == EPI_SWIGLU) {
        VSDE_CHECK_ARG(s_out && lds >= N / 2 && lds % 8 == 0 && ((uintptr_t)s_out % 16) == 0 && (!y || (ldy >= N && ldy % 8 == 0)),
                       VSDE_E_BADARG, "bad SwiGLU epilogue outputs");
        return launch_rows_k<EPI_SWIGLU>(p, st);
    }
    VSDE_CHECK_ARG(y && u_in && ldy >= 2 * N && ldu >= 2 * N && ldy % 8 == 0 && ldu % 8 == 0 && ((uintptr_t)y % 16) == 0 &&
                   ((uintptr_t)u_in % 16) == 0, VSDE_E_BADARG, "bad SwiGLU-backward epilogue buffers");
    return launch_rows_k<EPI_SWIGLU_BWD>(p, st);
}

extern "C" int vsde_linear_qknorm_bf16(const void *x, int64_t ldx, const void *w, const void *bias, int64_t M, int K, int heads,
                                       int gate_width, int tokens, const float *cosT, const float *sinT, const float *wq,
                                       const float *wk, const void *v0, const float *lam, double eps, void *q, void *k, void *v,
                                       void *gate, int64_t ldg, int gate_sigmoid, float *rinv, void *vdiff, void *stream) {
    VSDE_CHECK_ARG(x && w && q && k && v && cosT && sinT && wq && wk && M > 0 && heads > 0 && tokens > 0, VSDE_E_BADARG,
                   "bad linear_qknorm arguments");
    VSDE_CHECK_ARG((K == 256 || K == 128) && gate_width % 64 == 0 && gate_width >= 0 && (gate_width == 0 || (gate && ldg >= gate_width && ldg % 8 == 0)),
                   VSDE_E_BADARG, "linear_qknorm is built for K in {128, 256}, head_dim 64 and a gate block that is a multiple of 64 wide");
    VSDE_CHECK_ARG((!v0) == (!lam), VSDE_E_BADARG, "residual values and their mixing weight go together");
    VSDE_CHECK_ARG(ldx >= K && ldx % 8 == 0 && ((uintptr_t)x % 16) == 0 && ((uintptr_t)w % 16) == 0 && ((uintptr_t)q % 16) == 0 &&
                   ((uintptr_t)k % 16) == 0 && ((uintptr_t)v % 16) == 0 && ((uintptr_t)cosT % 16) == 0 && ((uintptr_t)sinT % 16) == 0,
                   VSDE_E_BADARG, "linear_qknorm operands must be 16-byte aligned");
    LinParams p = {};
    p.A = (const uint16_t *)x; p.lda = ldx; p.W = (const uint16_t *)w; p.bias = (const uint16_t *)bias;
    p.M = M; p.N = 3 * heads * 64 + gate_width; p.K = K;
    p.Qo = (uint16_t *)q; p.Ko = (uint16_t *)k; p.Vo = (uint16_t *)v; p.Go = (uint16_t *)gate; p.ldg = ldg;
    p.cosT = cosT; p.sinT = sinT; p.wq = wq; p.wk = wk; p.lam = lam; p.V0 = (const uint16_t *)v0;
    p.heads = heads; p.tokens = tokens; p.eps = (float)eps;
    VSDE_CHECK_ARG(!vdiff || (v0 && ((uintptr_t)vdiff % 16) == 0), VSDE_E_BADARG, "vdiff needs residual values (and 16-byte alignment)");
    p.Rinv = rinv; p.Vdiff = (uint16_t *)vdiff; p.gate_sigmoid = gate_sigmoid;
    return launch_qknorm(p, (hipStream_t)stream);
}

extern "C" int vsde_linear_gated_bf16(const void *attn, int64_t ldx, const void *gate, int64_t ldgate, const void *w, const void *bias,
                                      void *y, int64_t ldy, int64_t M, int N, int K, void *stream) {
    VSDE_CHECK_ARG(attn && gate && w && y && M > 0 && N > 0, VSDE_E_BADARG, "bad linear_gated arguments");
    VSDE_CHECK_ARG((K == 128 || K == 256) && N % 64 == 0, VSDE_E_BADARG, "linear_gated runs on the rows kernel: K in {128, 256}, N %% 64 == 0");
    VSDE_CHECK_ARG(ldx >= K && ldx % 8 == 0 && ldgate >= 64 && ldgate % 8 == 0 && ldy >= N && ldy % 8 == 0 && ((uintptr_t)attn % 16) == 0 &&
                   ((uintptr_t)gate % 16) == 0 && ((uintptr_t)w % 16) == 0 && ((uintptr_t)y % 16) == 0, VSDE_E_BADARG,
                   "linear_gated operands must be 16-byte aligned with row pitches that are multiples of 8 elements");
    LinParams p = {};
    p.A = (const uint16_t *)attn; p.lda = ldx; p.W = (const uint16_t *)w; p.bias = (const uint16_t *)bias;
    p.C = (uint16_t *)y; p.ldc = ldy; p.M = M; p.N = N; p.K = K; p.Gate = (const uint16_t *)gate; p.ldgate = ldgate;
    return launch_rows_k<EPI_PLAIN>(p, (hipStream_t)stream);
}

extern "C" int vsde_linear_gate_bwd_bf16(const void *dy, int64_t ldy, const void *w_t, const void *og, const void *s, int64_t lds,
                                         void *dattn, void *dgate, int64_t ldd, float *delta, int64_t M, int K, int heads, int tokens,
                                         void *stream) {
    VSDE_CHECK_ARG(dy && w_t && og && s && dattn && dgate && delta && M > 0 && heads > 0 && tokens > 0, VSDE_E_BADARG, "bad linear_gate_bwd arguments");
    VSDE_CHECK_ARG(K == 128 || K == 256, VSDE_E_BADARG, "linear_gate_bwd runs on the rows kernel: K in {128, 256}");
    VSDE_CHECK_ARG(ldy >= K && ldy % 8 == 0 && lds >= 64 && lds % 8 == 0 && ldd >= 64 && ldd % 8 == 0 && ((uintptr_t)dy % 16) == 0 &&
                   ((uintptr_t)w_t % 16) == 0 && ((uintptr_t)og % 16) == 0 && ((uintptr_t)s % 16) == 0 && ((uintptr_t)dattn % 16) == 0 &&
                   ((uintptr_t)dgate % 16) == 0, VSDE_E_BADARG,
                   "linear_gate_bwd operands must be 16-byte aligned with row pitches that are multiples of 8 elements");
    LinParams p = {};
    p.A = (const uint16_t *)dy; p.lda = ldy; p.W = (const uint16_t *)w_t; p.bias = nullptr;
    p.C = (uint16_t *)dattn; p.ldc = (int64_t)heads * 64; p.M = M; p.N = heads * 64; p.K = K;
    p.Og = (const uint16_t *)og; p.Sg = (const uint16_t *)s; p.ldsg = lds; p.Dgate = (uint16_t *)dgate; p.lddg = ldd; p.Delta = delta;
    p.heads = heads; p.tokens = tokens;
    return K == 128 ? launch_rows<128, EPI_GATE_BWD>(p, (hipStream_t)stream) : launch_rows<256, EPI_GATE_BWD>(p, (hipStream_t)stream);
}
```

viforsdes_amd/primitives/attn.py:

```python
from __future__ import annotations

from typing import Optional

import torch
from torch import Tensor, nn
from torch.nn import functional as F

from contextlib import nullcontext

from . import fused
from .embeddings import RotarySpec, apply_rope_1d
from .initializer import init_linear_, zero_linear_
from .norm import RMS


def _sdpa_backend_context(t: Tensor):
    if not t.is_cuda:
        return nullcontext()
    try:
        from torch.nn.attention import SDPBackend, sdpa_kernel
        return sdpa_kernel([SDPBackend.EFFICIENT_ATTENTION, SDPBackend.FLASH_ATTENTION, SDPBackend.MATH], set_priority=True)
    except Exception:
        return nullcontext()


def _sdpa(q: Tensor, k: Tensor, v: Tensor) -> Tensor:
    with _sdpa_backend_context(q):
        return F.scaled_dot_product_attention(q, k, v, dropout_p=0.0)


class Attention(nn.Module):
    def __init__(self, embed_dim: int, num_heads: int, *, qk_norm_eps: float = 1e-6, qk_norm: bool = True,
                 bias: bool = True, gate: bool = True, residual_v: bool = False) -> None:
        super().__init__()
        if embed_dim % num_heads:
            raise ValueError("embed_dim must be divisible by num_heads")
        self.embed_dim, self.num_heads, self.head_dim = embed_dim, num_heads, embed_dim // num_heads
        self.qkv_proj = init_linear_(nn.Linear(embed_dim, 3 * embed_dim, bias=bias))
        self.out_proj = init_linear_(nn.Linear(embed_dim, embed_dim, bias=bias))
        self._use_gate = gate
        if gate:
            self.gate_proj = zero_linear_(nn.Linear(embed_dim, self.head_dim, bias=True))
        self._use_residual_v = residual_v
        if residual_v:
            self.v_residual_lambda = nn.Parameter(torch.tensor(0.5))
        make_norm = (lambda: RMS(self.head_dim, eps=qk_norm_eps, requires_grad=False)) if qk_norm else nn.Identity
        self.q_norm, self.k_norm = make_norm(), make_norm()

    def fusable(self, hidden_states: Tensor, rotary: Optional[RotarySpec]) -> bool:
        return (fused.ENABLED and rotary is not None and self._use_gate and isinstance(self.q_norm, RMS)
                and not self.q_norm.weight.requires_grad and not self.k_norm.weight.requires_grad
                and fused.usable(hidden_states, self.embed_dim, self.head_dim))

    def forward_fused(self, hidden_states: Tensor, *, rotary: RotarySpec, v0: Optional[Tensor],
                      v0link: Optional["fused.GradLink"] = None, defer_out: bool = False) -> tuple[Tensor, Tensor]:
        N = hidden_states.shape[1]
        cos, sin = rotary.cos_sin_tables(N)
        mix = self._use_residual_v and v0 is not None
        lin = fused.linear
        n_out = self.qkv_proj.weight.shape[0] + self.gate_proj.weight.shape[0]
        if fused.packed_linear_usable(hidden_states, n_out, self.embed_dim):
            pack = getattr(self, "_proj_pack", None)
            if pack is None or pack.weight.device != hidden_states.device:
                has_b = self.qkv_proj.bias is not None
                pack = fused.row_pack([self.qkv_proj.weight, self.gate_proj.weight],
                                      [self.qkv_proj.bias, self.gate_proj.bias] if has_b else None)
                object.__setattr__(self, "_proj_pack", pack)
            if fused.attention_core_usable(hidden_states, pack, self.num_heads, self.head_dim, self.q_norm.weight, self.k_norm.weight, cos):
                out, v = fused.attention_core(hidden_states, pack, cos, sin, self.q_norm.weight, self.k_norm.weight,
                                              v0.transpose(1, 2) if mix else None, self.v_residual_lambda if mix else None,
                                              self.num_heads, self.q_norm.eps, self.head_dim ** -0.5, v0link,
                                              out_pack=fused.plain_pack(self.out_proj.weight, self.out_proj.bias))
                return out, v.transpose(1, 2)
            if fused.projection_split_nograd_usable(hidden_states, pack, self.num_heads, self.head_dim, self.q_norm.weight, cos):
                q, k, v, glog = fused.projection_split_nograd(hidden_states, pack, cos, sin, self.q_norm.weight, self.k_norm.weight,
                                                              v0.transpose(1, 2) if mix else None,
                                                              self.v_residual_lambda if mix else None, self.num_heads,
                                                              self.q_norm.eps)
                if fused.attention_usable(q):
                    out_tm = fused.attention(q, k, v, self.head_dim ** -0.5)
                else:
                    out_tm = _sdpa(q.transpose(1, 2), k.transpose(1, 2), v.transpose(1, 2)).transpose(1, 2)
                B_, N_ = hidden_states.shape[0], hidden_states.shape[1]
                if glog.shape[-1] == 64 and self.head_dim == 64 and self.out_proj.weight.shape[0] % 64 == 0:
                    po = fused.plain_pack(self.out_proj.weight, self.out_proj.bias)
                    if defer_out and fused.BLOCK_OUT_PROJ and self.out_proj.weight.shape[0] == self.embed_dim:
                        return (fused.DeferredOutProjection(out_tm.contiguous().view(B_, N_, self.embed_dim), glog.reshape(B_ * N_, 64), po),
                                v.transpose(1, 2))
                    wo, bo = po.operands()
                    y_out = fused._hip.linear_gated_bf16(out_tm.contiguous().view(B_ * N_, self.embed_dim), glog.reshape(B_ * N_, 64), wo, bo)
                    return y_out.view(B_, N_, -1), v.transpose(1, 2)
                merged = fused._hip.gate_merge_fwd(out_tm.contiguous(), glog, True)
                return lin(merged, self.out_proj.weight, self.out_proj.bias), v.transpose(1, 2)
            y = fused.packed_linear(hidden_states, pack)
        else:
            W = torch.cat([self.qkv_proj.weight, self.gate_proj.weight], dim=0)
            b = torch.cat([self.qkv_proj.bias, self.gate_proj.bias], dim=0) if self.qkv_proj.bias is not None else None
            y = lin(hidden_states, W, b)
        link = fused.GradLink()
        q, k, v = fused.attention_projection_split(y, cos, sin, self.q_norm.weight, self.k_norm.weight,
                                                   v0.transpose(1, 2) if mix else None,
                                                   self.v_residual_lambda if mix else None, self.num_heads,
                                                   self.q_norm.eps, True, link, v0link)
        if fused.attention_usable(q):
            out_tm = fused.attention(q, k, v, self.head_dim ** -0.5)
        else:
            out_tm = _sdpa(q.transpose(1, 2), k.transpose(1, 2), v.transpose(1, 2)).transpose(1, 2)
        merged = fused.gate_merge_joint(out_tm, y, self.num_heads, True, link)
        return lin(merged, self.out_proj.weight, self.out_proj.bias), v.transpose(1, 2)

    def forward(self, hidden_states: Tensor, *, rotary: Optional[RotarySpec] = None, v0: Optional[Tensor] = None,
                return_value: bool = False):
        B, N, _ = hidden_states.shape
        q, k, v = self.qkv_proj(hidden_states).view(B, N, 3, self.num_heads, self.head_dim).unbind(dim=2)
        q, k = self.q_norm(q), self.k_norm(k)
        q, k, v = q.transpose(1, 2), k.transpose(1, 2), v.transpose(1, 2)
        if rotary is not None:
            q, k = apply_rope_1d(q, rotary.rotary_freqs), apply_rope_1d(k, rotary.rotary_freqs)
        if self._use_residual_v and v0 is not None:
            if v0.shape != v.shape:
                raise ValueError(f"v0 shape {tuple(v0.shape)} must match value heads {tuple(v.shape)}")
            lam = self.v_residual_lambda
            v = lam * v + (1.0 - lam) * v0
        out = _sdpa(q, k, v)
        if self._use_gate:
            out = out * torch.sigmoid(self.gate_proj(hidden_states)).unsqueeze(1)
        out = self.out_proj(out.transpose(1, 2).reshape(B, N, self.embed_dim))
        if self._use_residual_v or return_value:
            return out, v
        return out
```

viforsdes_amd/primitives/fused.py:

```python
from __future__ import annotations

import os
import weakref
from typing import Optional

import torch
from torch import Tensor
from torch.autograd.function import once_differentiable

from .. import _hip

ENABLED = True


def fp16_autocast() -> bool:
    return torch.is_autocast_enabled() and torch.get_autocast_dtype("cuda") == torch.float16


def usable(x: Tensor, channels: int, head_dim: int) -> bool:
    half = head_dim // 2
    return (x.is_cuda and x.dtype in (torch.float32, torch.bfloat16) and not fp16_autocast() and channels % 64 == 0 and channels <= 1024
            and head_dim % 2 == 0 and 1 <= half <= 64 and (half & (half - 1)) == 0)


# ... 95 lines not shown
        if self.grad is None:
            self.grad = torch.zeros_like(self.allm)
        o = (6 * block + j) * self.C
        return self.grad[:, o:o + self.C]

    def take_grad(self) -> Tensor:
        g, self.grad = (self.grad if self.grad is not None else torch.zeros_like(self.allm)), None
        return g


class _LnModulateM(torch.autograd.Function):
    @staticmethod
    def forward(ctx, x, allm, mods, sc, sh, eps, final, link=None):
        x = x.contiguous()
        y, mean, rstd = _hip.ln_modulate_fwd(x, mods.vec(*sc), mods.vec(*sh), eps)
        ctx.save_for_backward(x, mean, rstd)
        ctx.meta = (mods, sc, sh, final, link)
        return y

    @staticmethod
    @once_differentiable
    def backward(ctx, dy):
        x, mean, rstd = ctx.saved_tensors
        mods, sc, sh, final, link = ctx.meta
        dres = link.take() if link is not None else None
        dx, _, _ = _hip.ln_modulate_bwd(x, mods.vec(*sc), dy.to(x.dtype).contiguous(), mean, rstd, dres,
                                        dscale=mods.gvec(*sc), dshift=mods.gvec(*sh))
        return dx, (mods.take_grad() if final else None), None, None, None, None, None, None


class _ResidualNormM(torch.autograd.Function):
    @staticmethod
    def forward(ctx, x, y, allm, mods, gt, sc, sh, eps, link=None):
        x = x.contiguous(); y = y.to(x.dtype).contiguous()
        xnew, h, mean, rstd = _hip.residual_ln_fwd(x, y, mods.vec(*gt), mods.vec(*sc), mods.vec(*sh), eps)
        ctx.save_for_backward(xnew, y, mean, rstd)
        ctx.meta = (mods, gt, sc, sh, link)
        return xnew, h

    @staticmethod
    @once_differentiable
    def backward(ctx, dxnew, dh):
        xnew, y, mean, rstd = ctx.saved_tensors
        mods, gt, sc, sh, link = ctx.meta
        dh = torch.zeros_like(xnew) if dh is None else dh.to(xnew.dtype).contiguous()
        dxnew = None if dxnew is None else dxnew.to(xnew.dtype).contiguous()
        dx, dy, _, _, _ = _hip.residual_ln_bwd(xnew, y, mods.vec(*gt), mods.vec(*sc), dh, dxnew, mean, rstd,
                                               dgate=mods.gvec(*gt), dscale=mods.gvec(*sc), dshift=mods.gvec(*sh))
        if link is not None and ctx.needs_input_grad[0]:
            link.value, dx = dx, None
        return dx, dy, None, None, None, None, None, None, None


class _GatedResidualM(torch.autograd.Function):
    @staticmethod
    def forward(ctx, x, y, allm, mods, gt):
        x = x.contiguous(); y = y.to(x.dtype).contiguous()
        ctx.save_for_backward(y)
        ctx.meta = (mods, gt)
        return _hip.gated_residual_fwd(x, y, mods.vec(*gt))

    @staticmethod
    @once_differentiable
    def backward(ctx, dout):
        (y,) = ctx.saved_tensors
        mods, gt = ctx.meta
        dout = dout.to(y.dtype).contiguous()
        dy, _ = _hip.gated_residual_bwd(y, mods.vec(*gt), dout, dgate=mods.gvec(*gt))
        return dout, dy, None, None, None


def ln_modulate_m(x: Tensor, mods: Modulations, scale: tuple[int, int], shift: tuple[int, int], eps: float, final: bool = False,
                  link: Optional[GradLink] = None) -> Tensor:
    return _LnModulateM.apply(x, mods.allm, mods, scale, shift, eps, final, link)


def residual_norm_m(x: Tensor, y: Tensor, mods: Modulations, gate: tuple[int, int], scale: tuple[int, int], shift: tuple[int, int],
                    eps: float, link: Optional[GradLink] = None) -> tuple[Tensor, Tensor]:
    return _ResidualNormM.apply(x, y, mods.allm, mods, gate, scale, shift, eps, link)


def gated_residual_m(x: Tensor, y: Tensor, mods: Modulations, gate: tuple[int, int]) -> Tensor:
    return _GatedResidualM.apply(x, y, mods.allm, mods, gate)


class _SwiGLU(torch.autograd.Function):
    @staticmethod
    def forward(ctx, u):
        u = u.contiguous()
        ctx.save_for_backward(u)
        return _hip.swiglu_fwd(u)

    @staticmethod
    @once_differentiable
    def backward(ctx, dout):
        (u,) = ctx.saved_tensors
        return _hip.swiglu_bwd(u, dout.to(u.dtype).contiguous())


def swiglu(u: Tensor) -> Tensor:
    return _SwiGLU.apply(u)


class _GateMerge(torch.autograd.Function):
    @staticmethod
    def forward(ctx, attn, glog, token_major):
        attn, glog = attn.contiguous(), glog.to(attn.dtype).contiguous()
        ctx.save_for_backward(attn, glog)
        ctx.token_major = token_major
        return _hip.gate_merge_fwd(attn, glog, token_major)

    @staticmethod
    @once_differentiable
    def backward(ctx, dout):
        attn, glog = ctx.saved_tensors
        dattn, dglog = _hip.gate_merge_bwd(attn, glog, dout.to(attn.dtype).contiguous(), ctx.token_major)
        return dattn, dglog, None


def gate_merge(attn: Tensor, gate_logits: Tensor, token_major: bool = False) -> Tensor:
    return _GateMerge.apply(attn, gate_logits, token_major)


class _GateMergeJoint(torch.autograd.Function):

    @staticmethod
    def forward(ctx, attn, y, off, token_major, link):
        attn = attn.contiguous()
        ctx.save_for_backward(attn, y)
        ctx.meta = (off, token_major, link)
        d = attn.shape[-1]
        return _hip.gate_merge_fwd(attn, y[..., off:off + d], token_major)

    @staticmethod
    @once_differentiable
    def backward(ctx, dout):
        attn, y = ctx.saved_tensors
        off, token_major, link = ctx.meta
        d = attn.shape[-1]
        dy = torch.empty_like(y) if off + d == y.shape[-1] else torch.zeros_like(y)
        dattn, _ = _hip.gate_merge_bwd(attn, y[..., off:off + d], dout.to(attn.dtype).contiguous(), token_major,
                                       dglog=dy[..., off:off + d])
        link.value = dy
        return dattn, None, None, None, None


class _QkNormRopeJoint(torch.autograd.Function):
    @staticmethod
    def forward(ctx, y, cos, sin, wq, wk, v0, lam, heads, eps, token_major, width, link, v0link):
        v0c = v0.to(y.dtype).contiguous() if v0 is not None else None
        lamc = lam.detach().float().reshape(1).contiguous() if lam is not None else None
        q, k, v = _hip.qk_norm_rope_fwd(y[..., :width], cos, sin, wq, wk, v0c, lamc, heads, eps, token_major)
        ctx.save_for_backward(y, cos, sin, wq, wk, v0c, lamc)
        ctx.meta = (heads, eps, lam.dtype if lam is not None else None, token_major, width, link, v0link)
        return q, k, v

    @staticmethod
    @once_differentiable
    def backward(ctx, dq, dk, dv):
        y, cos, sin, wq, wk, v0, lam = ctx.saved_tensors
        heads, eps, lam_dtype, token_major, width, link, v0link = ctx.meta
        dy = link.take()
        if dy is None:
            dy = torch.zeros_like(y)
        c = lambda t: t.to(y.dtype).contiguous()
        acc = v0link.value if (v0link is not None and v0 is not None) else None
# ... 593 lines not shown
def deep256(x2: Tensor, pack: PackedWeight, transposed: bool, bias: Optional[Tensor]) -> Tensor:
    attr = "_deep_image_t" if transposed else "_deep_image"
    img = getattr(pack, attr, None)
    if img is None:
        img = DeepImage(pack, transposed)
        setattr(pack, attr, img)
    return _hip.linear_deep256(x2, img.operand(), bias)


class DeferredOutProjection:

    def __init__(self, attn: Tensor, glog: Tensor, pack: PackedWeight) -> None:
        self.attn, self.glog, self.pack = attn, glog, pack


class MlpBwdImages:

    def __init__(self, pin: PackedWeight, pout: PackedWeight, width: int) -> None:
        assert pin.grad_rows is not None, "the fused backward works on the 16-row interleaved u / du layout"
        C, TP, dev = pin.weight.shape[1], width // 32, pin.weight.device
        self.nbytes = _hip.mlp_bwd_image_bytes(C)
        self.w2_elems = 32 * (C + 8)
        w2_bytes = (32 * (2 * C + 16) + 1023) // 1024 * 1024
        self.w1_off = w2_bytes // 2
        self.img = torch.zeros(TP, self.nbytes // 2, device=dev, dtype=torch.bfloat16)
        ks, h, e = torch.meshgrid(torch.arange(4), torch.arange(2), torch.arange(8), indexing="ij")
        ab, q, gp, i = ks >> 1, ks & 1, e >> 2, e & 3
        unit = 8 * (2 * q + gp) + 4 * h + i
        rows = 32 * (unit // 16) + 16 * ab + unit % 16
        self.rows = (64 * torch.arange(TP)[:, None] + rows.reshape(1, -1)).reshape(-1).to(dev)
        self.packs, self.width, self.C, self.TP = (pin, pout), width, C, TP
        self._key = None
        PackedWeight._derived.add(self)

    @torch.no_grad()
    def refresh_if_stale(self) -> None:
        pin, pout = self.packs
        key = (tuple(pin._versions or ()), tuple(pout._versions or ()))
        if key == self._key:
            return
        C, TP = self.C, self.TP
        self.img[:, :self.w2_elems].view(TP, 32, C + 8)[:, :, :C].copy_(pout.weight.t().reshape(TP, 32, C))
        w1 = pin.weight.index_select(0, self.rows).view(TP, 4, 2, 8, C).permute(0, 1, 2, 4, 3)
        self.img[:, self.w1_off:self.w1_off + 4 * 2 * C * 8].view(TP, 4, 2, C, 8).copy_(w1)
        self._key = key

    def operand(self) -> Tensor:
        for pk in self.packs:
            pk.operands()
        self.refresh_if_stale()
        return self.img


def mlp_block_nograd_usable(x: Tensor, mods: Optional["Modulations"], width: int) -> bool:
    return (ENABLED and OWN_GEMM and FUSED_MLP and BLOCK_MLP and not torch.is_grad_enabled() and mods is not None and x.is_cuda
            and x.dtype == torch.bfloat16 and x.ndim == 3 and x.shape[-1] in (128, 256) and width % 64 == 0 and width >= 64
            and x.shape[1] >= 86 and x.numel() // x.shape[-1] >= BLOCK_MLP_MIN_ROWS and mods.allm.dtype == torch.bfloat16)


@torch.no_grad()
def mlp_block_nograd(x: Tensor, attn_out, mods: "Modulations", block: int, nxt: Optional[int], eps: float, eps_next: float,
                     pin: PackedWeight, pout: PackedWeight):
    img = getattr(pin, "_mlp_images", None)
    if img is None:
        img = pin._mlp_images = MlpImages(pin, pout, pout.weight.shape[1])
    w1i, w2i, b1i = img.operands()
    sn = None if nxt is None else mods.vec(nxt, 0)
    hs = None if nxt is None else mods.vec(nxt, 1)
    if isinstance(attn_out, DeferredOutProjection):
        po = attn_out.pack
        oimg = getattr(po, "_out_image", None)
        if oimg is None:
            oimg = po._out_image = OutProjImage(po)
        return _hip.mlp_attn_block_fwd(x.contiguous(), attn_out.attn, attn_out.glog, oimg.operand(), po.bias, mods.vec(block, 2),
                                       mods.vec(block, 3), mods.vec(block, 4), mods.vec(block, 5), sn, hs, eps, eps_next, w1i, w2i, b1i,
                                       pout.bias, pout.weight.shape[1])
    return _hip.mlp_block_fwd(x.contiguous(), attn_out.to(x.dtype).contiguous(), mods.vec(block, 2), mods.vec(block, 3), mods.vec(block, 4),
                              mods.vec(block, 5), sn, hs, eps, eps_next, w1i, w2i, b1i, pout.bias, pout.weight.shape[1])


class _SwiGLUMLP(torch.autograd.Function):

    @staticmethod
    def forward(ctx, x, pin, pout, train, *params):
        w1, b1 = pin.operands()
        w2, b2 = pout.operands()
        x2 = x.reshape(-1, x.shape[-1]).contiguous()
        if not train and FUSED_MLP and x2.shape[1] in (128, 256) and w2.shape[1] % 64 == 0 and x2.shape[0] >= BLOCK_MLP_MIN_ROWS:
            img = getattr(pin, "_mlp_images", None)
            if img is None:
                img = pin._mlp_images = MlpImages(pin, pout, w2.shape[1])
            w1i, w2i, b1i = img.operands()
            y, _ = _hip.mlp_fwd(x2, w1i, w2i, b1i, b2, w2.shape[1])
            return y.reshape(*x.shape[:-1], w2.shape[0])
        u, s_ = _hip.linear_swiglu_bf16(x2, w1, b1, want_u=train)
        y = deep256(s_, pout, False, b2) if deep256_usable(s_.shape[0], w2.shape[0], w2.shape[1]) else _mm_nt(s_, w2, b2)
        if train:
            ctx.save_for_backward(x2, u, s_, w1)
        ctx.packs = (pin, pout)
        ctx.xshape = x.shape
        return y.reshape(*x.shape[:-1], w2.shape[0])

    @staticmethod
    @once_differentiable
    def backward(ctx, dy):
        x2, u, s_, w1 = ctx.saved_tensors
        pin, pout = ctx.packs
        dy2 = dy.to(torch.bfloat16).reshape(-1, dy.shape[-1]).contiguous()
        if (FUSED_MLP_BWD and pin.grad_rows is not None and dy2.shape[1] in (128, 256) and pout.weight.shape[1] % 64 == 0
                and dy2.shape[0] >= BLOCK_MLP_MIN_ROWS and _hip.has_ablations()):
            img = getattr(pin, "_mlp_bwd_images", None)
            if img is None:
                img = pin._mlp_bwd_images = MlpBwdImages(pin, pout, pout.weight.shape[1])
            du, dx = _hip.mlp_bwd(dy2, u, img.operand(), pout.weight.shape[1])
        else:
            du = _hip.linear_swiglu_bwd_bf16(dy2, pout.transposed(), u)
            if deep256_usable(du.shape[0], w1.shape[1], w1.shape[0]):
                dx = deep256(du, pin, True, None)
            elif own_gemm(du.shape[0], w1.shape[1], w1.shape[0]):
                dx = _hip.linear_bf16(du, pin.transposed(), None)
            else:
                dx = du @ w1
        g1 = _pack_weight_grads(du, x2, pin, pin.grad_row_map, None if pin.grad_rows is None else pin.grad_rows.numel())
        g2 = _pack_weight_grads(dy2, s_, pout)
        return (dx.reshape(ctx.xshape), None, None, None, *g1, *g2)


def swiglu_mlp_usable(x: Tensor, width: int) -> bool:
    rows = x.numel() // x.shape[-1]
    return (x.is_cuda and x.dtype == torch.bfloat16 and own_gemm(rows, 2 * width, x.shape[-1], _hip.EPI_SWIGLU)
            and own_gemm(rows, width, x.shape[-1], _hip.EPI_SWIGLU_BWD))


def swiglu_mlp(x: Tensor, pin: PackedWeight, pout: PackedWeight) -> Tensor:
    train = torch.is_grad_enabled() and (x.requires_grad or any(q.requires_grad for q in pin.params + pout.params))
    return _SwiGLUMLP.apply(x, pin, pout, train, *pin.params, *pout.params)


ATTN_FUSED_TRAIN = os.environ.get("VSDE_ATTN_FUSED_TRAIN", "1") != "0"
GATE_BWD_GEMM = os.environ.get("VSDE_GATE_BWD_GEMM", "1") != "0"
_NONZERO: dict[int, tuple] = {}


def _all_nonzero(w: Tensor) -> bool:
    hit = _NONZERO.get(id(w))
    if hit is not None and hit[0]() is w and hit[1] == w._version:
        return hit[2]
    ok = bool((w.detach() != 0).all())
    _NONZERO[id(w)] = (weakref.ref(w), w._version, ok)
    return ok


class _AttentionCore(torch.autograd.Function):

    @staticmethod
    def forward(ctx, x, pack, opack, cos, sin, wq, wk, v0, lam, heads, eps, scale, v0link, *params):
        B, N, K = x.shape
        w, b = pack.operands()
        mix = v0 is not None
        v0c = v0.to(torch.bfloat16).contiguous() if mix else None
        lamc = lam.detach().float().reshape(1).contiguous() if mix else None
        x2 = x.reshape(B * N, K)
        q, k, v, glog, rinv, vdiff = _hip.linear_qknorm_bf16(x2, w, b, heads, N, cos, sin, wq, wk, v0c, lamc, eps, save=True)
        shape = (B, N, heads, 64)
        og, lse = _hip.attention_fwd_gated(q.view(shape), k.view(shape), v.view(shape), glog, scale)
        ctx.save_for_backward(x2, q, k, v, glog, og, lse, rinv, vdiff, cos, sin, wq, wk, lamc)
        ctx.meta = (pack, opack, heads, scale, lam.dtype if mix else None, v0link, (B, N, K))
        ctx.set_materialize_grads(False)
        if opack is None:
            return og.view(B, N, heads * 64), v.view(shape)
        wo, bo = opack.operands()
        return _mm_nt(og.view(B * N, heads * 64), wo, bo).view(B, N, wo.shape[0]), v.view(shape)

    @staticmethod
    @once_differentiable
    def backward(ctx, dout, dv_out):
        x2, q, k, v, glog, og, lse, rinv, vdiff, cos, sin, wq, wk, lamc = ctx.saved_tensors
        pack, opack, heads, scale, lam_dtype, v0link, (B, N, K) = ctx.meta
        M, C, C3, G = B * N, heads * 64, 3 * heads * 64, glog.shape[1]
        shape = (B, N, heads, 64)
        mix = vdiff is not None
        dy = torch.empty(M, C3 + G, device=x2.device, dtype=torch.bfloat16)
        ograds: tuple = ()
        if opack is None:
            dmerged = torch.zeros(M, C, device=x2.device, dtype=torch.bfloat16) if dout is None else dout.to(torch.bfloat16).reshape(M, C)
            dattn, delta = _hip.gate_bwd_delta(dmerged.contiguous().view(shape), og, glog, dy[:, C3:])
        else:
            wo = opack.weight
            do2 = (torch.zeros(M, wo.shape[0], device=x2.device, dtype=torch.bfloat16) if dout is None
                   else dout.to(torch.bfloat16).reshape(M, wo.shape[0]).contiguous())
            if GATE_BWD_GEMM and wo.shape[0] in (128, 256) and own_gemm(M, C, wo.shape[0]):
                dattn, delta = _hip.linear_gate_bwd(do2, opack.transposed(), og, glog, dy[:, C3:], N)
            else:
                dattn, delta = _hip.gate_bwd_delta((do2 @ wo).view(shape), og, glog, dy[:, C3:])
            ograds = tuple(_pack_weight_grads(do2, og.view(M, C), opack))
        acc = v0link.value if (v0link is not None and mix) else None
        extra = v0link.take() if (v0link is not None and not mix) else None
        if dv_out is not None:
            dv_out = dv_out.to(torch.bfloat16).contiguous()
            extra = dv_out if extra is None else (extra + dv_out)
        dv0, dlam = _hip.attention_bwd_fused(dattn, q.view(shape), k.view(shape), v.view(shape), lse, delta, rinv, cos, sin, wq, wk,
                                             vdiff, lamc, acc, extra, dy, scale)
        if v0link is not None and mix:
            v0link.value, dv0 = dv0, None
        if dlam is not None:
            dlam = dlam.to(lam_dtype).reshape(())
        wb = pack.weight
        dx = None
        if ctx.needs_input_grad[0]:
            if deep256_usable(M, wb.shape[1], wb.shape[0]):
                dx = deep256(dy, pack, True, None).view(B, N, K)
            else:
                dx = (_hip.linear_bf16(dy, pack.transposed(), None) if own_gemm(M, wb.shape[1], wb.shape[0]) else dy @ wb).view(B, N, K)
        return (dx, None, None, None, None, None, None, dv0, dlam, None, None, None, None, *_pack_weight_grads(dy, x2.contiguous(), pack), *ograds)


def attention_core_usable(x: Tensor, pack: "PackedWeight", heads: int, d: int, wq: Tensor, wk: Tensor, cos: Tensor) -> bool:
    rows = x.numel() // x.shape[-1]
    return (ENABLED and OWN_GEMM and ATTN_FUSED_TRAIN and torch.is_grad_enabled() and x.is_cuda and x.dtype == torch.bfloat16
            and x.ndim == 3 and x.shape[-1] in (128, 256) and d == 64 and pack.weight.shape[0] == 3 * heads * 64 + 64 and rows >= OWN_GEMM_MIN_ROWS
            and wq.dtype == torch.float32 and wk.dtype == torch.float32 and cos.dtype == torch.float32 and cos.shape[-1] == 32
            and _hip.attention_fused_supported(x.shape[1], d) and _all_nonzero(wq) and _all_nonzero(wk))


def attention_core(x: Tensor, pack: "PackedWeight", cos: Tensor, sin: Tensor, wq: Tensor, wk: Tensor, v0: Optional[Tensor],
                   lam: Optional[Tensor], heads: int, eps: float, scale: float, v0link: Optional[GradLink],
                   out_pack: Optional["PackedWeight"] = None):
    oparams = () if out_pack is None else tuple(out_pack.params)
    return _AttentionCore.apply(x, pack, out_pack, cos.contiguous(), sin.contiguous(), wq.contiguous(), wk.contiguous(), v0,
                                lam if v0 is not None else None, heads, eps, scale, v0link, *pack.params, *oparams)


def row_pack(weights: list[Tensor], biases: Optional[list[Tensor]], pad_to: Optional[int] = None) -> PackedWeight:
    rows = sum(w.shape[0] for w in weights)
    wp, bp, r = [], [], 0
    for i, w in enumerate(weights):
        wp.append((w, 0, w.shape[0], r))
        if biases is not None:
            bp.append((biases[i], 0, w.shape[0], r))
        r += w.shape[0]
    return PackedWeight(pad_to or rows, weights[0].shape[1], wp, bp or None, weights[0].device)


def swiglu_packs(w_in: Tensor, b_in: Optional[Tensor], w_out: Tensor, b_out: Optional[Tensor], width: int,
                 interleave: bool = False):
    h = w_out.shape[1]
    if interleave:
        wp, bp, rows = [], [], []
        for half in (0, 1):
            for j0 in range(0, h, 16):
                n, dst = min(16, h - j0), 32 * (j0 // 16) + 16 * half
                wp.append((w_in, half * h + j0, n, dst))
                if b_in is not None:
                    bp.append((b_in, half * h + j0, n, dst))
                rows.extend(range(dst, dst + n))
        pin = PackedWeight(2 * width, w_in.shape[1], wp, bp or None, w_in.device,
                           grad_rows=torch.tensor(rows, device=w_in.device, dtype=torch.long))
    else:
        pin = PackedWeight(2 * width, w_in.shape[1], [(w_in, 0, h, 0), (w_in, h, h, width)],
                           None if b_in is None else [(b_in, 0, h, 0), (b_in, h, h, width)], w_in.device)
    n = w_out.shape[0]
    pout = PackedWeight(n, width, [(w_out, 0, n, 0)], None if b_out is None else [(b_out, 0, n, 0)], w_out.device)
    return pin, pout
```

viforsdes_amd/primitives/mlp.py:

```python
from __future__ import annotations

import torch
from torch import Tensor, nn
from torch.nn import functional as F

from . import fused
from .initializer import init_linear_


_PAD = 128 if __import__("os").environ.get("VSDE_MLP_PAD") == "128" else 64


class SwiGLU(nn.Module):
    def __init__(self, in_dim: int, hidden_dim: int, *, bias: bool = True) -> None:
        super().__init__()
        self.in_dim, self.hidden_dim = in_dim, hidden_dim
        self.input_proj = init_linear_(nn.Linear(in_dim, 2 * hidden_dim, bias=bias))
        self.output_proj = init_linear_(nn.Linear(hidden_dim, in_dim, bias=bias))

    def _padded_weights(self, width: int):
        h, pad = self.hidden_dim, width - self.hidden_dim
        w1 = F.pad(self.input_proj.weight.view(2, h, self.in_dim), (0, 0, 0, pad)).reshape(2 * width, self.in_dim)
        b1 = None if self.input_proj.bias is None else F.pad(self.input_proj.bias.view(2, h), (0, pad)).reshape(2 * width)
        return w1, b1, F.pad(self.output_proj.weight, (0, pad))

    def padded_width(self) -> int:
        return -(-self.hidden_dim // _PAD) * _PAD

    def packs(self, x: Tensor, fused_mlp: bool):
        width = self.padded_width()
        packs = getattr(self, "_packs", None)
        if (packs is None or packs[0].weight.device != x.device or packs[0].weight.shape[0] != 2 * width
                or (packs[0].grad_rows is not None) != fused_mlp):
            packs = fused.swiglu_packs(self.input_proj.weight, self.input_proj.bias, self.output_proj.weight,
                                       self.output_proj.bias, width, interleave=fused_mlp)
            object.__setattr__(self, "_packs", packs)
        return packs

    def forward(self, x: Tensor) -> Tensor:
        if fused.ENABLED and x.is_cuda and x.dtype in (torch.float32, torch.bfloat16) and not fused.fp16_autocast():
            width = self.padded_width()
            if fused.packed_linear_usable(x, 2 * width, self.in_dim):
                fused_mlp = fused.swiglu_mlp_usable(x, width)
                packs = self.packs(x, fused_mlp)
                if fused_mlp:
                    return fused.swiglu_mlp(x, packs[0], packs[1])
                return fused.packed_linear(fused.swiglu(fused.packed_linear(x, packs[0])), packs[1])
            if width != self.hidden_dim:
                w1, b1, w2 = self._padded_weights(width)
                return fused.linear(fused.swiglu(fused.linear(x, w1, b1)), w2, self.output_proj.bias)
            return fused.linear(fused.swiglu(fused.linear(x, self.input_proj.weight, self.input_proj.bias)),
                                self.output_proj.weight, self.output_proj.bias)
        a, b = self.input_proj(x).chunk(2, dim=-1)
        return self.output_proj(F.silu(a) * b)
```

viforsdes_amd/primitives/sit.py:

```python
from __future__ import annotations

from dataclasses import dataclass
from typing import Optional

import torch
from torch import Tensor, nn

from . import fused
from .attn import Attention
from .cond import CondBranch, CondModulator
from .embeddings import RotarySpec
from .initializer import init_linear_
from .mlp import SwiGLU
from .norm import LayerNormConfig


@dataclass(frozen=True)
class SiTConfig:
    in_dim: int
    hidden_dim: int
    out_dim: int
    cond_dim: int
    num_heads: int
    depth: int
# ... 9 lines not shown

class SiTBlock(nn.Module):
    def __init__(self, *, dim: int, num_heads: int, mlp_hidden_dim: int, cond_dim: int, bias: bool = True,
                 attn_gate: bool = True, attn_residual_v: bool = False, use_qk_norm: bool = True,
                 qk_norm_eps: float = 1e-6, attn_norm: LayerNormConfig = LayerNormConfig(affine=False),
                 mlp_norm: LayerNormConfig = LayerNormConfig(affine=False)) -> None:
        super().__init__()
        self.dim, self.num_heads = dim, num_heads
        self._cond_modulator = CondModulator(cond_dim=cond_dim, hidden_dim=dim, branches=2)
        self.self_attn = Attention(dim, num_heads, bias=bias, gate=attn_gate, qk_norm=use_qk_norm,
                                   qk_norm_eps=qk_norm_eps, residual_v=attn_residual_v)
        self.mlp = SwiGLU(dim, mlp_hidden_dim, bias=bias)
        self.attn_norm = attn_norm.build(dim=dim)
        self.mlp_norm = mlp_norm.build(dim=dim)

    def cond_params(self, *, cond: Tensor) -> tuple[CondBranch, ...]:
        return self._cond_modulator(cond=cond)

    def fusable(self, hidden_states: Tensor, cond: Tensor, rotary: Optional[RotarySpec]) -> bool:
        plain = lambda n: isinstance(n, nn.LayerNorm) and not n.elementwise_affine
        return cond.ndim == 2 and plain(self.attn_norm) and plain(self.mlp_norm) and self.self_attn.fusable(hidden_states, rotary)

    def forward(self, hidden_states: Tensor, *, cond: Tensor, rotary: Optional[RotarySpec] = None,
                v0: Optional[Tensor] = None) -> tuple[Tensor, Tensor]:
        if self.fusable(hidden_states, cond, rotary):
            sa, ha, ga, sm, hm, gm = self._cond_modulator.net(cond).chunk(6, dim=-1)
            link1, link2 = fused.GradLink(), fused.GradLink()
            h1 = fused.ln_modulate(hidden_states, sa, ha, self.attn_norm.eps, link1)
            attn_out, values = self.self_attn.forward_fused(h1, rotary=rotary, v0=v0)
            hidden_states = fused.gated_residual(hidden_states, attn_out, ga, link1)
            h2 = fused.ln_modulate(hidden_states, sm, hm, self.mlp_norm.eps, link2)
            return fused.gated_residual(hidden_states, self.mlp(h2), gm, link2), values
        if cond.ndim == 2:
            cond = cond.unsqueeze(1)
        attn_mod, mlp_mod = self.cond_params(cond=cond)
        attn_out, values = self.self_attn(attn_mod.affine(self.attn_norm(hidden_states)), rotary=rotary, v0=v0,
                                          return_value=True)
        hidden_states = hidden_states + attn_mod.gate(attn_out)
        mlp_out = self.mlp(mlp_mod.affine(self.mlp_norm(hidden_states)))
        return hidden_states + mlp_mod.gate(mlp_out), values


class SiT(nn.Module):
    def __init__(self, config: SiTConfig) -> None:
        super().__init__()
        self.config = config
        self.blocks = nn.ModuleList([
            SiTBlock(dim=config.hidden_dim, num_heads=config.num_heads, mlp_hidden_dim=config.mlp_hidden_dim,
                     cond_dim=config.cond_dim, bias=config.bias, attn_gate=config.attn_gate,
                     attn_residual_v=config.attn_residual_v and idx > 0, use_qk_norm=config.use_qk_norm,
                     qk_norm_eps=config.qk_norm_eps, attn_norm=config.attn_norm, mlp_norm=config.mlp_norm)
            for idx in range(config.depth)])
        self.input_proj = init_linear_(nn.Linear(config.in_dim, config.hidden_dim, bias=config.bias))
        self.output_proj = init_linear_(nn.Linear(config.hidden_dim, config.out_dim, bias=config.bias))

    def _packed_modulations(self, cond: Tensor) -> Optional["fused.Modulations"]:
        nets = [blk._cond_modulator.net for blk in self.blocks]
        lin = [n[1] for n in nets]
        per = lin[0].weight.shape[0]
        C = self.config.hidden_dim
        if not (cond.is_cuda and cond.dtype == torch.bfloat16 and fused.ENABLED and all(isinstance(n[0], nn.SiLU) for n in nets)
                and all(l.bias is not None and l.weight.shape[0] == 6 * C for l in lin) and C % 8 == 0 and cond.shape[-1] % 8 == 0):
            return None
        pack = getattr(self, "_mods_pack", None)
        if pack is None or pack.weight.device != cond.device:
            pack = fused.row_pack([l.weight for l in lin], [l.bias for l in lin])
            object.__setattr__(self, "_mods_pack", pack)
        return fused.Modulations(fused.packed_linear(torch.nn.functional.silu(cond), pack), C)

    def _forward_fused_chain(self, tokens: Tensor, cond: Tensor, rotary: RotarySpec) -> Tensor:
        blocks = self.blocks
        nb = len(blocks)
        tokens = tokens.contiguous()
        mods = self._packed_modulations(cond)
        SA, HA, GA, SM, HM, GM = range(6)
        link0 = fused.GradLink()
        if mods is None:
            ml = [blk._cond_modulator.net(cond).chunk(6, dim=-1) for blk in blocks]
            h1 = fused.ln_modulate(tokens, ml[0][SA], ml[0][HA], blocks[0].attn_norm.eps, link0)
        else:
            h1 = fused.ln_modulate_m(tokens, mods, (0, SA), (0, HA), blocks[0].attn_norm.eps, final=True, link=link0)
        v0: Optional[Tensor] = None
        v0link = fused.GradLink() if self.config.attn_residual_v else None
        for k, blk in enumerate(blocks):
            block_form = (isinstance(blk.mlp, SwiGLU) and blk.mlp.input_proj.bias is not None
                          and fused.mlp_block_nograd_usable(tokens, mods, blk.mlp.padded_width())
                          and fused.swiglu_mlp_usable(tokens, blk.mlp.padded_width()))
            attn_out, values = blk.self_attn.forward_fused(h1, rotary=rotary, v0=v0, v0link=v0link, defer_out=block_form)
            if v0 is None and self.config.attn_residual_v:
                v0 = values
            lk = link0 if k == 0 else None
            if block_form:
                pin, pout = blk.mlp.packs(tokens, True)
                tokens, h1 = fused.mlp_block_nograd(tokens, attn_out, mods, k, k + 1 if k + 1 < nb else None, blk.mlp_norm.eps,
                                                    blocks[k + 1].attn_norm.eps if k + 1 < nb else blk.mlp_norm.eps, pin, pout)
                continue
            if mods is None:
                x1, h2 = fused.residual_norm(tokens, attn_out, ml[k][GA], ml[k][SM], ml[k][HM], blk.mlp_norm.eps, lk)
            else:
                x1, h2 = fused.residual_norm_m(tokens, attn_out, mods, (k, GA), (k, SM), (k, HM), blk.mlp_norm.eps, lk)
            mlp_out = blk.mlp(h2)
            if k + 1 < nb:
                eps = blocks[k + 1].attn_norm.eps
                if mods is None:
                    tokens, h1 = fused.residual_norm(x1, mlp_out, ml[k][GM], ml[k + 1][SA], ml[k + 1][HA], eps)
                else:
                    tokens, h1 = fused.residual_norm_m(x1, mlp_out, mods, (k, GM), (k + 1, SA), (k + 1, HA), eps)
            else:
                tokens = (fused.gated_residual(x1, mlp_out, ml[k][GM]) if mods is None
                          else fused.gated_residual_m(x1, mlp_out, mods, (k, GM)))
        return tokens

    def forward(self, x: Tensor, *, cond: Tensor, rotary: Optional[RotarySpec] = None, row_tokens: Optional[Tensor] = None) -> Tensor:
        if x.ndim == 3 and x.stride(0) == 0 and x.shape[0] > 1:
            row = row_tokens if (row_tokens is not None and row_tokens.shape == x.shape[1:]) else x[0]
            tokens = self.input_proj(row).unsqueeze(0).expand(x.shape[0], -1, -1)
        else:
            tokens = self.input_proj(x)
        if all(block.fusable(tokens, cond, rotary) for block in self.blocks):
            return fused.linear(self._forward_fused_chain(tokens, cond, rotary), self.output_proj.weight, self.output_proj.bias)
        v0: Optional[Tensor] = None
        for block in self.blocks:
            tokens, values = block(tokens, cond=cond, rotary=rotary, v0=v0)
            if v0 is None and self.config.attn_residual_v:
                v0 = values
        return fused.linear(tokens, self.output_proj.weight, self.output_proj.bias)
```

Measured before the change: 19760.

## Fuse gated-residual LayerNorm modulation into the prologue of the QKV and SwiGLU GEMMs

Adds a LayerNorm prologue to the row-GEMM kernel. The gated residual add, LN statistics and scale/shift modulation are computed on the A-fragments already staged in LDS, and the result feeds the QK-norm attention projection and the SwiGLU input projection directly. The goal is to drop the separate residual_norm kernel launch and the round trip of the normalised activations through global memory. The kernel still writes the new residual stream, the mean/rstd and optionally h, which are needed for backward, and the fused path only handles K = 256. The encoder forward chain is rewired to defer each residual-norm as a pending prologue for the next projection, with backward routed through the prologue object.

```diff
diff --git a/include/vsde_hip.h b/include/vsde_hip.h
--- a/include/vsde_hip.h
+++ b/include/vsde_hip.h
@@ -165,6 +165,15 @@
                             int tokens, const float *cosT, const float *sinT, const float *wq, const float *wk, const void *v0,
                             const float *lam, double eps, void *q, void *k, void *v, void *gate, int64_t ldg, int gate_sigmoid,
                             float *rinv, void *vdiff, void *stream);
+int vsde_linear_qknorm_ln_bf16(const void *x, const void *y, const void *ln_gate, const void *ln_scale, const void *ln_shift,
+                               int64_t mod_pitch, double ln_eps, void *xnew, void *h, float *mean, float *rstd, const void *w,
+                               const void *bias, int64_t M, int K, int heads, int gate_width, int tokens, const float *cosT,
+                               const float *sinT, const float *wq, const float *wk, const void *v0, const float *lam, double eps,
+                               void *q, void *k, void *v, void *gate, int64_t ldg, int gate_sigmoid, float *rinv, void *vdiff,
+                               void *stream);
+int vsde_linear_swiglu_ln_bf16(const void *x, const void *y, const void *ln_gate, const void *ln_scale, const void *ln_shift,
+                               int64_t mod_pitch, double ln_eps, int tokens, void *xnew, void *h, float *mean, float *rstd,
+                               const void *w, const void *bias, void *u, void *s_out, int64_t M, int N, int K, void *stream);
 int vsde_linear_gated_bf16(const void *attn, int64_t ldx, const void *gate, int64_t ldgate, const void *w, const void *bias, void *y,
                            int64_t ldy, int64_t M, int N, int K, void *stream);
 
diff --git a/viforsdes_amd/_hip.py b/viforsdes_amd/_hip.py
--- a/viforsdes_amd/_hip.py
+++ b/viforsdes_amd/_hip.py
@@ -54,7 +54,7 @@
     "vsde_attention_max_tokens", "vsde_attention_fwd_bf16", "vsde_attention_bwd_bf16",
     "vsde_attention_fused_supported", "vsde_attention_fwd_gated_bf16", "vsde_gate_bwd_delta", "vsde_attention_bwd_fused_partials",
     "vsde_attention_bwd_fused_bf16",
-    "vsde_euler_maruyama_fwd", "vsde_euler_maruyama_bwd", "vsde_sde_coefficients_fwd", "vsde_sde_coefficients_bwd", "vsde_linear_bf16_supported", "vsde_linear_bf16", "vsde_linear_qknorm_bf16", "vsde_linear_gated_bf16", "vsde_linear_gate_bwd_bf16",
+    "vsde_euler_maruyama_fwd", "vsde_euler_maruyama_bwd", "vsde_sde_coefficients_fwd", "vsde_sde_coefficients_bwd", "vsde_linear_bf16_supported", "vsde_linear_bf16", "vsde_linear_qknorm_bf16", "vsde_linear_qknorm_ln_bf16", "vsde_linear_swiglu_ln_bf16", "vsde_linear_gated_bf16", "vsde_linear_gate_bwd_bf16",
     "vsde_mlp_image_bytes", "vsde_mlp_fwd_bf16", "vsde_mlp_block_fwd_bf16", "vsde_mlp_attn_block_fwd_bf16", "vsde_linear_deep256_bf16", "vsde_mlp_debug_trace", "vsde_wgrad_debug_trace", "vsde_attn_debug_trace", "vsde_mlp_bwd_image_bytes", "vsde_mlp_bwd_bf16",
     "vsde_pack_tile_bytes", "vsde_pack_refresh", "vsde_optim_chunk_bytes", "vsde_optim_chunk_elems", "vsde_optim_step",
 )
@@ -783,6 +783,50 @@
     return q, k, v, gate
 
 
+def _ln_prologue_args(x, y, gate, scale, shift, eps, want_h):
+    dev = _require_hip(x, y, gate, scale, shift)
+    if x.dtype != torch.bfloat16 or y.dtype != torch.bfloat16 or x.ndim != 3 or y.shape != x.shape or not (x.is_contiguous() and y.is_contiguous()):
+        raise ValueError("the LayerNorm prologue needs contiguous bf16 x, y [B,N,C] of one shape")
+    B, N, C = x.shape
+    xnew = torch.empty_like(x); h = torch.empty_like(x) if want_h else None
+    mean = torch.empty(B * N, device=dev, dtype=torch.float32); rstd = torch.empty_like(mean)
+    args = (_ptr(x), _ptr(y), _ptr(gate), _ptr(scale), _ptr(shift), _i64(_mod_pitch(C, gate, scale, shift)), ctypes.c_double(eps))
+    return args, xnew, h, mean, rstd
+
+
+def linear_qknorm_ln_bf16(x, y, gate, scale, shift, ln_eps, w, bias, heads, cos, sin, wq, wk, v0, lam, eps, want_h=True):
+    lib = load()
+    args, xnew, h, mean, rstd = _ln_prologue_args(x, y, gate, scale, shift, ln_eps, want_h)
+    dev = _require_hip(w, cos, sin, wq, wk)
+    B, N, K = x.shape
+    M, C = B * N, heads * 64
+    G = w.shape[0] - 3 * C
+    q = torch.empty(M, C, device=dev, dtype=torch.bfloat16); k = torch.empty_like(q); v = torch.empty_like(q)
+    g = torch.empty(M, G, device=dev, dtype=torch.bfloat16) if G > 0 else None
+    rinv = torch.empty(M, 2 * heads, device=dev, dtype=torch.float32)
+    vdiff = torch.empty(M, C, device=dev, dtype=torch.bfloat16) if v0 is not None else None
+    with torch.cuda.device(dev):
+        _call(lib.vsde_linear_qknorm_ln_bf16, *args, _ptr(xnew), _ptr(h), _ptr(mean), _ptr(rstd), _ptr(w), _ptr(bias), _i64(M),
+              ctypes.c_int(K), ctypes.c_int(heads), ctypes.c_int(G), ctypes.c_int(N), _ptr(cos), _ptr(sin), _ptr(wq), _ptr(wk), _ptr(v0),
+              _ptr(lam), ctypes.c_double(eps), _ptr(q), _ptr(k), _ptr(v), _ptr(g), _i64(G), ctypes.c_int(1), _ptr(rinv), _ptr(vdiff),
+              _stream(dev))
+    return xnew, h, mean, rstd, q, k, v, g, rinv, vdiff
+
+
+def linear_swiglu_ln_bf16(x, y, gate, scale, shift, ln_eps, w, bias, want_h=True):
+    lib = load()
+    args, xnew, h, mean, rstd = _ln_prologue_args(x, y, gate, scale, shift, ln_eps, want_h)
+    dev = _require_hip(w)
+    B, T, K = x.shape
+    M, N = B * T, w.shape[0]
+    u = torch.empty(M, N, device=dev, dtype=torch.bfloat16)
+    s = torch.empty(M, N // 2, device=dev, dtype=torch.bfloat16)
+    with torch.cuda.device(dev):
+        _call(lib.vsde_linear_swiglu_ln_bf16, *args, ctypes.c_int(T), _ptr(xnew), _ptr(h), _ptr(mean), _ptr(rstd), _ptr(w), _ptr(bias),
+              _ptr(u), _ptr(s), _i64(M), ctypes.c_int(N), ctypes.c_int(K), _stream(dev))
+    return xnew, h, mean, rstd, u, s
+
+
 def attention_fused_supported(N: int, head_dim: int) -> bool:
     return bool(load().vsde_attention_fused_supported(ctypes.c_int(N), ctypes.c_int(head_dim)))
 
diff --git a/viforsdes_amd/csrc/vsde_common.h b/viforsdes_amd/csrc/vsde_common.h
--- a/viforsdes_amd/csrc/vsde_common.h
+++ b/viforsdes_amd/csrc/vsde_common.h
@@ -100,6 +100,12 @@
 __device__ __forceinline__ float xor_lane(float v) {
     static_assert(K > 0 && K < 32, "ds_swizzle bit mode reaches the 32 lanes of a half wave");
     return __int_as_float(__builtin_amdgcn_ds_swizzle(__float_as_int(v), (K << 10) | 0x1f));
+}
+
+template <typename RND>
+__device__ __forceinline__ float ln_residual_elem(float x, float gate, float y, RND rnd) { return rnd(x + rnd(gate * y)); }
+__device__ __forceinline__ float ln_modulate_elem(float v, float mu, float rs, float scale, float shift) {
+    return (v - mu) * rs * (1.0f + scale) + shift;
 }
 
 __device__ __forceinline__ float wave_sum(float v) {
diff --git a/viforsdes_amd/csrc/vsde_encoder.hip b/viforsdes_amd/csrc/vsde_encoder.hip
--- a/viforsdes_amd/csrc/vsde_encoder.hip
+++ b/viforsdes_amd/csrc/vsde_encoder.hip
@@ -107,7 +107,7 @@
                     float rg[V];
                     Pack<T, V>::load(res_gate + b * mp + (sl * LPR + lane) * V, rg);
 #pragma unroll
-                    for (int e = 0; e < V; ++e) v[sl][e] = rnd<T>(v[sl][e] + rnd<T>(rg[e] * ry[sl][e]));
+                    for (int e = 0; e < V; ++e) v[sl][e] = ln_residual_elem(v[sl][e], rg[e], ry[sl][e], [](float a) { return rnd<T>(a); });
                     Pack<T, V>::store(xnew + m * C + (sl * LPR + lane) * V, v[sl]);
                 }
 #pragma unroll
@@ -129,7 +129,7 @@
                 float sc[V], sh[V], o[V];
                 Pack<T, V>::load(scale + b * mp + c, sc); Pack<T, V>::load(shift + b * mp + c, sh);
 #pragma unroll
-                for (int e = 0; e < V; ++e) o[e] = (v[sl][e] - mu) * rs * (1.0f + sc[e]) + sh[e];
+                for (int e = 0; e < V; ++e) o[e] = ln_modulate_elem(v[sl][e], mu, rs, sc[e], sh[e]);
                 Pack<T, V>::store(y + m * C + c, o);
             }
 #pragma unroll
diff --git a/viforsdes_amd/csrc/vsde_linear.hip b/viforsdes_amd/csrc/vsde_linear.hip
--- a/viforsdes_amd/csrc/vsde_linear.hip
+++ b/viforsdes_amd/csrc/vsde_linear.hip
@@ -34,6 +34,8 @@
     const uint16_t *Gate; int64_t ldgate;
     int dbg;
     int xstage;
+    const uint16_t *Ry, *Lgate, *Lscale, *Lshift; int64_t lmp; float leps;
+    uint16_t *Xnew, *Hout; float *Lmean, *Lrstd;
 };
 
 typedef __bf16 hwbf16x2 __attribute__((ext_vector_type(2)));
@@ -377,7 +379,130 @@
     __builtin_amdgcn_s_setprio(0);
 }
 
-template <int KC, int EPI, int NKH, int NW>
+template <int KS>
+__device__ __forceinline__ float ln_group_tree(float (&g)[KS]) {
+#pragma unroll
+    for (int off = KS / 2; off > 0; off >>= 1)
+#pragma unroll
+        for (int i = 0; i < off; ++i) g[i] = g[i] + g[i + off];
+    return sum_xor32(g[0]);
+}
+
+template <int KT> __device__ __forceinline__ int xs_seg(int rl, int lc) { return rl * (KT * 2) + ((lc ^ (rl & 15)) << 4); }
+template <int KT> __device__ __forceinline__ int xs_frag(int r, int hf, int ks) { return r * (KT * 2) + (((hf + 2 * ks) ^ (r & 15)) << 4); }
+
+template <int KT>
+__device__ __forceinline__ void ln_frag_store(const bf16x8 (&a)[KT / 16], char *xs, uint16_t *dst, int64_t rowb, int64_t M, int lane) {
+    constexpr int KS = KT / 16, CPR = KT / 8, RPI = 64 / CPR;
+    asm volatile("" : "+v"(lane));
+    const int r = lane & 31, hf = lane >> 5, lrow = lane / CPR, lc = lane % CPR;
+    wave_lds_fence();
+#pragma unroll
+    for (int ks = 0; ks < KS; ++ks) *(bf16x8 *)(xs + xs_frag<KT>(r, hf, ks)) = a[ks];
+    wave_lds_fence();
+    uint16_t *d = dst + (rowb + lrow) * KT + lc * 8;
+#pragma unroll
+    for (int i = 0; i < KS; ++i) {
+        const int rl = i * RPI + lrow;
+        const u32x4 v = *(const u32x4 *)(xs + xs_seg<KT>(rl, lc));
+        if (rowb + rl < M) __builtin_nontemporal_store(v, (u32x4 *)(d + i * RPI * KT));
+    }
+}
+
+template <int KT>
+__device__ __forceinline__ void ln_prologue(const LinParams &p, bf16x8 (&a)[KT / 16], char *xs, int64_t rowb, int lane, bool out) {
+    static_assert(KT == 256, "the statistics follow ln_mod_fwd_kernel's lane layout at C = 256");
+    constexpr int KS = KT / 16, CPR = KT / 8, RPI = 64 / CPR;
+    asm volatile("" : "+v"(lane), "+v"(rowb));
+    const int r = lane & 31, hf = lane >> 5, lrow = lane / CPR, lc = lane % CPR;
+    {
+        u32x4 t[KS];
+        const uint16_t *src = p.Ry + (rowb + lrow) * KT + lc * 8;
+#pragma unroll
+        for (int i = 0; i < KS; ++i)
+            t[i] = rowb + i * RPI + lrow < p.M ? *(const u32x4 *)(src + i * RPI * KT) : u32x4{0u, 0u, 0u, 0u};
+        wave_lds_fence();
+#pragma unroll
+        for (int i = 0; i < KS; ++i) *(u32x4 *)(xs + xs_seg<KT>(i * RPI + lrow, lc)) = t[i];
+        wave_lds_fence();
+    }
+    const int64_t m = rowb + r < p.M ? rowb + r : p.M - 1;
+    const int64_t bo = (int64_t)((int)m / p.tokens) * p.lmp + 8 * hf;
+    constexpr int G = 4, NG = KS / G;
+    auto fetch = [&](u32x4 (&d)[G], const uint16_t *vec, int grp) {
+#pragma unroll
+        for (int j = 0; j < G; ++j) d[j] = *(const u32x4 *)(vec + bo + (grp * G + j) * 16);
+    };
+    float gs[KS];
+    {
+        u32x4 gv[2][G];
+        fetch(gv[0], p.Lgate, 0);
+#pragma unroll
+        for (int grp = 0; grp < NG; ++grp) {
+            if (grp + 1 < NG) fetch(gv[(grp + 1) & 1], p.Lgate, grp + 1);
+            __builtin_amdgcn_sched_barrier(0);
+#pragma unroll
+            for (int j = 0; j < G; ++j) {
+                const int ks = grp * G + j;
+                const u32x4 x4 = __builtin_bit_cast(u32x4, a[ks]), y4 = *(const u32x4 *)(xs + xs_frag<KT>(r, hf, ks)), g4 = gv[grp & 1][j];
+                u32x4 o;
+                float s = 0.f;
+#pragma unroll
+                for (int e = 0; e < 4; ++e) {
+                    const float lo = ln_residual_elem(bf_lo(x4[e]), bf_lo(g4[e]), bf_lo(y4[e]), rbf);
+                    const float hi = ln_residual_elem(bf_hi(x4[e]), bf_hi(g4[e]), bf_hi(y4[e]), rbf);
+                    s += lo; s += hi;
+                    o[e] = pack_bf16x2(lo, hi);
+                }
+                a[ks] = __builtin_bit_cast(bf16x8, o);
+                gs[ks] = s;
+            }
+            __builtin_amdgcn_sched_barrier(0);
+        }
+    }
+    const float mu = ln_group_tree(gs) / p.K;
+#pragma unroll
+    for (int ks = 0; ks < KS; ++ks) {
+        const u32x4 x4 = __builtin_bit_cast(u32x4, a[ks]);
+        float q = 0.f;
+#pragma unroll
+        for (int e = 0; e < 4; ++e) {
+            const float dl = bf_lo(x4[e]) - mu; q += dl * dl;
+            const float dh = bf_hi(x4[e]) - mu; q += dh * dh;
+        }
+        gs[ks] = q;
+    }
+    const float rs = rsqrtf(ln_group_tree(gs) / p.K + p.leps);
+    if (out) {
+        if (hf == 0 && rowb + r < p.M) { p.Lmean[rowb + r] = mu; p.Lrstd[rowb + r] = rs; }
+        ln_frag_store<KT>(a, xs, p.Xnew, rowb, p.M, lane);
+    }
+    {
+        u32x4 sv[2][G], hv[2][G];
+        fetch(sv[0], p.Lscale, 0); fetch(hv[0], p.Lshift, 0);
+#pragma unroll
+        for (int grp = 0; grp < NG; ++grp) {
+            if (grp + 1 < NG) { fetch(sv[(grp + 1) & 1], p.Lscale, grp + 1); fetch(hv[(grp + 1) & 1], p.Lshift, grp + 1); }
+            __builtin_amdgcn_sched_barrier(0);
+#pragma unroll
+            for (int j = 0; j < G; ++j) {
+                const int ks = grp * G + j;
+                const u32x4 sc4 = sv[grp & 1][j], sh4 = hv[grp & 1][j];
+                u32x4 x4 = __builtin_bit_cast(u32x4, a[ks]), o;
+                asm volatile("" : "+v"(x4));
+#pragma unroll
+                for (int e = 0; e < 4; ++e)
+                    o[e] = pack_bf16x2(ln_modulate_elem(bf_lo(x4[e]), mu, rs, bf_lo(sc4[e]), bf_lo(sh4[e])),
+                                       ln_modulate_elem(bf_hi(x4[e]), mu, rs, bf_hi(sc4[e]), bf_hi(sh4[e])));
+                a[ks] = __builtin_bit_cast(bf16x8, o);
+            }
+            __builtin_amdgcn_sched_barrier(0);
+        }
+    }
+    if (out && p.Hout != nullptr) ln_frag_store<KT>(a, xs, p.Hout, rowb, p.M, lane);
+}
+
+template <int KC, int EPI, int NKH, int NW, bool PRO = false>
 __global__ void __launch_bounds__(64 * NW, NW == 4 ? 2 : 1) lin_rows_kernel(LinParams p) {
     constexpr int RB = rows_rb<EPI, NKH>(), ROWS = 32 * NW * RB, THREADS = 64 * NW;
     constexpr int KS = NKH * KC / 16, KT = NKH * KC, LDB = KC + 8, TILE = 33 * LDB;
@@ -394,7 +519,8 @@
     const int64_t row0 = stripe * ROWS + wave * (32 * RB);
 
     bf16x8 afr[RB][KS];
-    const bool xst = NKH == 1 && p.xstage && !(EPI == EPI_PLAIN && p.Gate != nullptr);
+    static_assert(!PRO || (NKH == 1 && KC == 256), "the LayerNorm prologue is built for K = 256");
+    const bool xst = PRO || (NKH == 1 && p.xstage && !(EPI == EPI_PLAIN && p.Gate != nullptr));
     if (xst) {
         constexpr int CPR = KT / 8, RPI = 64 / CPR;
         char *xs = (char *)lsm + wave * (32 * KT * 2);
@@ -417,6 +543,7 @@
             wave_lds_fence();
 #pragma unroll
             for (int ks = 0; ks < KS; ++ks) afr[rb][ks] = *(const bf16x8 *)(xs + r * (KT * 2) + (((h + 2 * ks) ^ (r & 15)) << 4));
+            if constexpr (PRO) ln_prologue<KT>(p, afr[rb], xs, row0 + rb * 32, lane, chunk == 0);
         }
         lds_barrier();
     }
@@ -766,10 +893,10 @@
 }
 template <int NB> static size_t cols_lds_bytes() { return (size_t)(2 * 32 * NB * C2_LDB) * sizeof(uint16_t); }
 
-template <int KC, int EPI, int NKH, int NW>
+template <int KC, int EPI, int NKH, int NW, bool PRO = false>
 static int launch_rows_nw(const LinParams &p, hipStream_t s) {
     const size_t lds = rows_lds_bytes<KC, EPI, NKH, NW>();
-    VSDE_CHECK_HIP(hipFuncSetAttribute((const void *)lin_rows_kernel<KC, EPI, NKH, NW>, hipFuncAttributeMaxDynamicSharedMemorySize, (int)lds));
+    VSDE_CHECK_HIP(hipFuncSetAttribute((const void *)lin_rows_kernel<KC, EPI, NKH, NW, PRO>, hipFuncAttributeMaxDynamicSharedMemorySize, (int)lds));
     constexpr int rows = 32 * NW * rows_rb<EPI, NKH>();
     constexpr int resident = NW == 4 ? 512 : 256;
     const int64_t stripes = (p.M + rows - 1) / rows;
@@ -821,7 +948,7 @@
     q.tail_local = (int)((groups - tail_groups) * chunks);
     q.tail_chunks = tail_chunks;
     const int64_t nwg = ((groups - tail_groups) * chunks + tail_groups * tail_chunks) * 8;
-    hipLaunchKernelGGL((lin_rows_kernel<KC, EPI, NKH, NW>), dim3((unsigned)nwg), dim3(64 * NW), lds, s, q);
+    hipLaunchKernelGGL((lin_rows_kernel<KC, EPI, NKH, NW, PRO>), dim3((unsigned)nwg), dim3(64 * NW), lds, s, q);
     VSDE_CHECK_HIP(hipGetLastError());
     return 0;
 }
@@ -940,10 +1067,35 @@
     return launch_rows_k<EPI_SWIGLU_BWD>(p, st);
 }
 
-extern "C" int vsde_linear_qknorm_bf16(const void *x, int64_t ldx, const void *w, const void *bias, int64_t M, int K, int heads,
-                                       int gate_width, int tokens, const float *cosT, const float *sinT, const float *wq,
-                                       const float *wk, const void *v0, const float *lam, double eps, void *q, void *k, void *v,
-                                       void *gate, int64_t ldg, int gate_sigmoid, float *rinv, void *vdiff, void *stream) {
+namespace vsde {
+struct LnPrologueArgs {
+    const void *y, *gate, *scale, *shift;
+    int64_t mod_pitch;
+    double eps;
+    void *xnew, *h;
+    float *mean, *rstd;
+};
+
+static bool al16(const void *ptr) { return ((uintptr_t)ptr % 16) == 0; }
+
+static int set_ln_prologue(LinParams &p, const LnPrologueArgs &a, int64_t ldx, int tokens) {
+    VSDE_CHECK_ARG(a.y && a.gate && a.scale && a.shift && a.xnew && a.mean && a.rstd, VSDE_E_BADARG, "bad LayerNorm prologue arguments");
+    VSDE_CHECK_ARG(p.K == 256 && ldx == p.K && tokens > 0 && p.M % tokens == 0 && p.M < ((int64_t)1 << 31), VSDE_E_BADARG,
+                   "the LayerNorm prologue needs K = 256, contiguous rows and M a multiple of tokens");
+    VSDE_CHECK_ARG(a.mod_pitch >= p.K && a.mod_pitch % 8 == 0 && al16(a.y) && al16(a.gate) && al16(a.scale) && al16(a.shift) &&
+                   al16(a.xnew) && (!a.h || al16(a.h)), VSDE_E_BADARG,
+                   "LayerNorm prologue operands must be 16-byte aligned with a modulation row pitch >= K that is a multiple of 8");
+    p.Ry = (const uint16_t *)a.y; p.Lgate = (const uint16_t *)a.gate; p.Lscale = (const uint16_t *)a.scale;
+    p.Lshift = (const uint16_t *)a.shift; p.lmp = a.mod_pitch; p.leps = (float)a.eps;
+    p.Xnew = (uint16_t *)a.xnew; p.Hout = (uint16_t *)a.h; p.Lmean = a.mean; p.Lrstd = a.rstd;
+    p.tokens = tokens;
+    return 0;
+}
+
+static int linear_qknorm(const LnPrologueArgs *ln, const void *x, int64_t ldx, const void *w, const void *bias, int64_t M, int K,
+                         int heads, int gate_width, int tokens, const float *cosT, const float *sinT, const float *wq, const float *wk,
+                         const void *v0, const float *lam, double eps, void *q, void *k, void *v, void *gate, int64_t ldg,
+                         int gate_sigmoid, float *rinv, void *vdiff, void *stream) {
     VSDE_CHECK_ARG(x && w && q && k && v && cosT && sinT && wq && wk && M > 0 && heads > 0 && tokens > 0, VSDE_E_BADARG,
                    "bad linear_qknorm arguments");
     VSDE_CHECK_ARG((K == 256 || K == 128) && gate_width % 64 == 0 && gate_width >= 0 && (gate_width == 0 || (gate && ldg >= gate_width && ldg % 8 == 0)),
@@ -960,7 +1112,44 @@
     p.heads = heads; p.tokens = tokens; p.eps = (float)eps;
     VSDE_CHECK_ARG(!vdiff || (v0 && ((uintptr_t)vdiff % 16) == 0), VSDE_E_BADARG, "vdiff needs residual values (and 16-byte alignment)");
     p.Rinv = rinv; p.Vdiff = (uint16_t *)vdiff; p.gate_sigmoid = gate_sigmoid;
+    if (ln) {
+        if (int rc = set_ln_prologue(p, *ln, ldx, tokens)) return rc;
+        return launch_rows_nw<256, EPI_QKNORM, 1, 4, true>(p, (hipStream_t)stream);
+    }
     return launch_qknorm(p, (hipStream_t)stream);
+}
+}
+
+extern "C" int vsde_linear_qknorm_bf16(const void *x, int64_t ldx, const void *w, const void *bias, int64_t M, int K, int heads,
+                                       int gate_width, int tokens, const float *cosT, const float *sinT, const float *wq,
+                                       const float *wk, const void *v0, const float *lam, double eps, void *q, void *k, void *v,
+                                       void *gate, int64_t ldg, int gate_sigmoid, float *rinv, void *vdiff, void *stream) {
+    return linear_qknorm(nullptr, x, ldx, w, bias, M, K, heads, gate_width, tokens, cosT, sinT, wq, wk, v0, lam, eps, q, k, v, gate, ldg,
+                         gate_sigmoid, rinv, vdiff, stream);
+}
+
+extern "C" int vsde_linear_qknorm_ln_bf16(const void *x, const void *y, const void *ln_gate, const void *ln_scale, const void *ln_shift,
+                                          int64_t mod_pitch, double ln_eps, void *xnew, void *h, float *mean, float *rstd, const void *w,
+                                          const void *bias, int64_t M, int K, int heads, int gate_width, int tokens, const float *cosT,
+                                          const float *sinT, const float *wq, const float *wk, const void *v0, const float *lam,
+                                          double eps, void *q, void *k, void *v, void *gate, int64_t ldg, int gate_sigmoid, float *rinv,
+                                          void *vdiff, void *stream) {
+    const LnPrologueArgs ln = {y, ln_gate, ln_scale, ln_shift, mod_pitch, ln_eps, xnew, h, mean, rstd};
+    return linear_qknorm(&ln, x, K, w, bias, M, K, heads, gate_width, tokens, cosT, sinT, wq, wk, v0, lam, eps, q, k, v, gate, ldg,
+                         gate_sigmoid, rinv, vdiff, stream);
+}
+
+extern "C" int vsde_linear_swiglu_ln_bf16(const void *x, const void *y, const void *ln_gate, const void *ln_scale, const void *ln_shift,
+                                          int64_t mod_pitch, double ln_eps, int tokens, void *xnew, void *h, float *mean, float *rstd,
+                                          const void *w, const void *bias, void *u, void *s_out, int64_t M, int N, int K, void *stream) {
+    VSDE_CHECK_ARG(x && w && s_out && M > 0 && N > 0 && N % 64 == 0, VSDE_E_BADARG, "bad linear_swiglu_ln arguments");
+    VSDE_CHECK_ARG(al16(x) && al16(w) && al16(s_out) && (!u || al16(u)), VSDE_E_BADARG, "linear_swiglu_ln operands must be 16-byte aligned");
+    LinParams p = {};
+    p.A = (const uint16_t *)x; p.lda = K; p.W = (const uint16_t *)w; p.bias = (const uint16_t *)bias;
+    p.C = (uint16_t *)u; p.ldc = N; p.S = (uint16_t *)s_out; p.lds_ = N / 2; p.M = M; p.N = N; p.K = K;
+    const LnPrologueArgs ln = {y, ln_gate, ln_scale, ln_shift, mod_pitch, ln_eps, xnew, h, mean, rstd};
+    if (int rc = set_ln_prologue(p, ln, K, tokens)) return rc;
+    return launch_rows_nw<256, EPI_SWIGLU, 1, 4, true>(p, (hipStream_t)stream);
 }
 
 extern "C" int vsde_linear_gated_bf16(const void *attn, int64_t ldx, const void *gate, int64_t ldgate, const void *w, const void *bias,
diff --git a/viforsdes_amd/primitives/attn.py b/viforsdes_amd/primitives/attn.py
--- a/viforsdes_amd/primitives/attn.py
+++ b/viforsdes_amd/primitives/attn.py
@@ -53,7 +53,8 @@
                 and fused.usable(hidden_states, self.embed_dim, self.head_dim))
 
     def forward_fused(self, hidden_states: Tensor, *, rotary: RotarySpec, v0: Optional[Tensor],
-                      v0link: Optional["fused.GradLink"] = None, defer_out: bool = False) -> tuple[Tensor, Tensor]:
+                      v0link: Optional["fused.GradLink"] = None, defer_out: bool = False,
+                      prologue: Optional["fused.LnPrologue"] = None) -> tuple:
         N = hidden_states.shape[1]
         cos, sin = rotary.cos_sin_tables(N)
         mix = self._use_residual_v and v0 is not None
@@ -67,11 +68,16 @@
                                       [self.qkv_proj.bias, self.gate_proj.bias] if has_b else None)
                 object.__setattr__(self, "_proj_pack", pack)
             if fused.attention_core_usable(hidden_states, pack, self.num_heads, self.head_dim, self.q_norm.weight, self.k_norm.weight, cos):
-                out, v = fused.attention_core(hidden_states, pack, cos, sin, self.q_norm.weight, self.k_norm.weight,
-                                              v0.transpose(1, 2) if mix else None, self.v_residual_lambda if mix else None,
-                                              self.num_heads, self.q_norm.eps, self.head_dim ** -0.5, v0link,
-                                              out_pack=fused.plain_pack(self.out_proj.weight, self.out_proj.bias))
-                return out, v.transpose(1, 2)
+                pro = prologue if (prologue is not None and fused.ln_prologue_usable(hidden_states)) else None
+                if prologue is not None and pro is None:
+                    return self._forward_materialised(prologue, rotary, v0, v0link, defer_out)
+                out, v, *xnew = fused.attention_core(hidden_states, pack, cos, sin, self.q_norm.weight, self.k_norm.weight,
+                                                     v0.transpose(1, 2) if mix else None, self.v_residual_lambda if mix else None,
+                                                     self.num_heads, self.q_norm.eps, self.head_dim ** -0.5, v0link,
+                                                     out_pack=fused.plain_pack(self.out_proj.weight, self.out_proj.bias), prologue=pro)
+                return (out, v.transpose(1, 2), *xnew)
+            if prologue is not None:
+                return self._forward_materialised(prologue, rotary, v0, v0link, defer_out)
             if fused.projection_split_nograd_usable(hidden_states, pack, self.num_heads, self.head_dim, self.q_norm.weight, cos):
                 q, k, v, glog = fused.projection_split_nograd(hidden_states, pack, cos, sin, self.q_norm.weight, self.k_norm.weight,
                                                               v0.transpose(1, 2) if mix else None,
@@ -94,6 +100,8 @@
                 return lin(merged, self.out_proj.weight, self.out_proj.bias), v.transpose(1, 2)
             y = fused.packed_linear(hidden_states, pack)
         else:
+            if prologue is not None:
+                return self._forward_materialised(prologue, rotary, v0, v0link, defer_out)
             W = torch.cat([self.qkv_proj.weight, self.gate_proj.weight], dim=0)
             b = torch.cat([self.qkv_proj.bias, self.gate_proj.bias], dim=0) if self.qkv_proj.bias is not None else None
             y = lin(hidden_states, W, b)
@@ -108,6 +116,11 @@
             out_tm = _sdpa(q.transpose(1, 2), k.transpose(1, 2), v.transpose(1, 2)).transpose(1, 2)
         merged = fused.gate_merge_joint(out_tm, y, self.num_heads, True, link)
         return lin(merged, self.out_proj.weight, self.out_proj.bias), v.transpose(1, 2)
+
+    def _forward_materialised(self, prologue: "fused.LnPrologue", rotary: RotarySpec, v0: Optional[Tensor],
+                              v0link: Optional["fused.GradLink"], defer_out: bool) -> tuple:
+        xnew, h = prologue.materialise()
+        return (*self.forward_fused(h, rotary=rotary, v0=v0, v0link=v0link, defer_out=defer_out), xnew)
 
     def forward(self, hidden_states: Tensor, *, rotary: Optional[RotarySpec] = None, v0: Optional[Tensor] = None,
                 return_value: bool = False):
diff --git a/viforsdes_amd/primitives/fused.py b/viforsdes_amd/primitives/fused.py
--- a/viforsdes_amd/primitives/fused.py
+++ b/viforsdes_amd/primitives/fused.py
@@ -201,6 +201,43 @@
 
 def gated_residual_m(x: Tensor, y: Tensor, mods: Modulations, gate: tuple[int, int]) -> Tensor:
     return _GatedResidualM.apply(x, y, mods.allm, mods, gate)
+
+
+LN_PROLOGUE = os.environ.get("VSDE_LN_PROLOGUE", "0") == "1"
+
+
+class LnPrologue:
+    __slots__ = ("x", "y", "mods", "gate", "scale", "shift", "eps", "link")
+
+    def __init__(self, x: Tensor, y: Tensor, mods: Modulations, gate: tuple[int, int], scale: tuple[int, int], shift: tuple[int, int],
+                 eps: float, link: Optional[GradLink] = None) -> None:
+        self.x, self.y, self.mods, self.gate, self.scale, self.shift, self.eps, self.link = x, y, mods, gate, scale, shift, eps, link
+
+    def materialise(self) -> tuple[Tensor, Tensor]:
+        return residual_norm_m(self.x, self.y, self.mods, self.gate, self.scale, self.shift, self.eps, self.link)
+
+    def forward_args(self) -> tuple:
+        m = self.mods
+        x = self.x.contiguous()
+        y = self.y.to(x.dtype).contiguous()
+        self.x = self.y = None
+        return x, y, m.vec(*self.gate), m.vec(*self.scale), m.vec(*self.shift)
+
+    def backward(self, xnew: Tensor, y: Tensor, mean: Tensor, rstd: Tensor, dh: Optional[Tensor], dxnew: Optional[Tensor],
+                 need_dx: bool) -> tuple[Optional[Tensor], Tensor]:
+        m = self.mods
+        dh = torch.zeros_like(xnew) if dh is None else dh.to(xnew.dtype).reshape(xnew.shape).contiguous()
+        dxnew = None if dxnew is None else dxnew.to(xnew.dtype).contiguous()
+        dx, dy, _, _, _ = _hip.residual_ln_bwd(xnew, y, m.vec(*self.gate), m.vec(*self.scale), dh, dxnew, mean, rstd,
+                                               dgate=m.gvec(*self.gate), dscale=m.gvec(*self.scale), dshift=m.gvec(*self.shift))
+        if self.link is not None and need_dx:
+            self.link.value, dx = dx, None
+        return dx, dy
+
+
+def ln_prologue_usable(x: Tensor) -> bool:
+    return (LN_PROLOGUE and ENABLED and torch.is_grad_enabled() and x.is_cuda and x.dtype == torch.bfloat16 and x.ndim == 3
+            and x.shape[-1] == 256)
 
 
 class _SwiGLU(torch.autograd.Function):
@@ -960,9 +997,19 @@
 class _SwiGLUMLP(torch.autograd.Function):
 
     @staticmethod
-    def forward(ctx, x, pin, pout, train, *params):
+    def forward(ctx, x, y, allm, pro, pin, pout, train, *params):
         w1, b1 = pin.operands()
         w2, b2 = pout.operands()
+        ctx.pro = pro
+        if pro is not None:
+            xs, ys, gt, sc, sh = pro.forward_args()
+            xnew, h, mean, rstd, u, s_ = _hip.linear_swiglu_ln_bf16(xs, ys, gt, sc, sh, pro.eps, w1, b1)
+            x2 = h.view(-1, h.shape[-1])
+            out = deep256(s_, pout, False, b2) if deep256_usable(s_.shape[0], w2.shape[0], w2.shape[1]) else _mm_nt(s_, w2, b2)
+            ctx.save_for_backward(x2, u, s_, w1, xnew, ys, mean, rstd)
+            ctx.packs = (pin, pout)
+            ctx.xshape = x.shape
+            return out.reshape(*x.shape[:-1], w2.shape[0]), xnew
         x2 = x.reshape(-1, x.shape[-1]).contiguous()
         if not train and FUSED_MLP and x2.shape[1] in (128, 256) and w2.shape[1] % 64 == 0 and x2.shape[0] >= BLOCK_MLP_MIN_ROWS:
             img = getattr(pin, "_mlp_images", None)
@@ -981,8 +1028,8 @@
 
     @staticmethod
     @once_differentiable
-    def backward(ctx, dy):
-        x2, u, s_, w1 = ctx.saved_tensors
+    def backward(ctx, dy, dxnew=None):
+        x2, u, s_, w1, *ln = ctx.saved_tensors
         pin, pout = ctx.packs
         dy2 = dy.to(torch.bfloat16).reshape(-1, dy.shape[-1]).contiguous()
         if (FUSED_MLP_BWD and pin.grad_rows is not None and dy2.shape[1] in (128, 256) and pout.weight.shape[1] % 64 == 0
@@ -1001,7 +1048,11 @@
                 dx = du @ w1
         g1 = _pack_weight_grads(du, x2, pin, pin.grad_row_map, None if pin.grad_rows is None else pin.grad_rows.numel())
         g2 = _pack_weight_grads(dy2, s_, pout)
-        return (dx.reshape(ctx.xshape), None, None, None, *g1, *g2)
+        if ctx.pro is not None:
+            xnew, y, mean, rstd = ln
+            dxs, dys = ctx.pro.backward(xnew, y, mean, rstd, dx, dxnew, ctx.needs_input_grad[0])
+            return (dxs, dys, None, None, None, None, None, *g1, *g2)
+        return (dx.reshape(ctx.xshape), None, None, None, None, None, None, *g1, *g2)
 
 
 def swiglu_mlp_usable(x: Tensor, width: int) -> bool:
@@ -1010,9 +1061,11 @@
             and own_gemm(rows, width, x.shape[-1], _hip.EPI_SWIGLU_BWD))
 
 
-def swiglu_mlp(x: Tensor, pin: PackedWeight, pout: PackedWeight) -> Tensor:
+def swiglu_mlp(x: Tensor, pin: PackedWeight, pout: PackedWeight, prologue: Optional[LnPrologue] = None):
     train = torch.is_grad_enabled() and (x.requires_grad or any(q.requires_grad for q in pin.params + pout.params))
-    return _SwiGLUMLP.apply(x, pin, pout, train, *pin.params, *pout.params)
+    if prologue is not None:
+        return _SwiGLUMLP.apply(x, prologue.y, prologue.mods.allm, prologue, pin, pout, True, *pin.params, *pout.params)
+    return _SwiGLUMLP.apply(x, None, None, None, pin, pout, train, *pin.params, *pout.params)
 
 
 ATTN_FUSED_TRAIN = os.environ.get("VSDE_ATTN_FUSED_TRAIN", "1") != "0"
@@ -1032,28 +1085,39 @@
 class _AttentionCore(torch.autograd.Function):
 
     @staticmethod
-    def forward(ctx, x, pack, opack, cos, sin, wq, wk, v0, lam, heads, eps, scale, v0link, *params):
+    def forward(ctx, x, y, allm, pro, pack, opack, cos, sin, wq, wk, v0, lam, heads, eps, scale, v0link, *params):
         B, N, K = x.shape
         w, b = pack.operands()
         mix = v0 is not None
         v0c = v0.to(torch.bfloat16).contiguous() if mix else None
         lamc = lam.detach().float().reshape(1).contiguous() if mix else None
-        x2 = x.reshape(B * N, K)
-        q, k, v, glog, rinv, vdiff = _hip.linear_qknorm_bf16(x2, w, b, heads, N, cos, sin, wq, wk, v0c, lamc, eps, save=True)
+        ln: tuple = ()
+        if pro is not None:
+            xs, ys, gt, sc, sh = pro.forward_args()
+            xnew, h, mean, rstd, q, k, v, glog, rinv, vdiff = _hip.linear_qknorm_ln_bf16(xs, ys, gt, sc, sh, pro.eps, w, b, heads, cos, sin,
+                                                                                        wq, wk, v0c, lamc, eps)
+            x2 = h.view(B * N, K)
+            ln = (xnew, ys, mean, rstd)
+        else:
+            x2 = x.reshape(B * N, K)
+            q, k, v, glog, rinv, vdiff = _hip.linear_qknorm_bf16(x2, w, b, heads, N, cos, sin, wq, wk, v0c, lamc, eps, save=True)
         shape = (B, N, heads, 64)
         og, lse = _hip.attention_fwd_gated(q.view(shape), k.view(shape), v.view(shape), glog, scale)
-        ctx.save_for_backward(x2, q, k, v, glog, og, lse, rinv, vdiff, cos, sin, wq, wk, lamc)
+        ctx.save_for_backward(x2, q, k, v, glog, og, lse, rinv, vdiff, cos, sin, wq, wk, lamc, *ln)
         ctx.meta = (pack, opack, heads, scale, lam.dtype if mix else None, v0link, (B, N, K))
+        ctx.pro = pro
         ctx.set_materialize_grads(False)
         if opack is None:
-            return og.view(B, N, heads * 64), v.view(shape)
-        wo, bo = opack.operands()
-        return _mm_nt(og.view(B * N, heads * 64), wo, bo).view(B, N, wo.shape[0]), v.view(shape)
-
-    @staticmethod
-    @once_differentiable
-    def backward(ctx, dout, dv_out):
-        x2, q, k, v, glog, og, lse, rinv, vdiff, cos, sin, wq, wk, lamc = ctx.saved_tensors
+            out = og.view(B, N, heads * 64)
+        else:
+            wo, bo = opack.operands()
+            out = _mm_nt(og.view(B * N, heads * 64), wo, bo).view(B, N, wo.shape[0])
+        return (out, v.view(shape), *ln[:1])
+
+    @staticmethod
+    @once_differentiable
+    def backward(ctx, dout, dv_out, dxnew=None):
+        x2, q, k, v, glog, og, lse, rinv, vdiff, cos, sin, wq, wk, lamc, *ln = ctx.saved_tensors
         pack, opack, heads, scale, lam_dtype, v0link, (B, N, K) = ctx.meta
         M, C, C3, G = B * N, heads * 64, 3 * heads * 64, glog.shape[1]
         shape = (B, N, heads, 64)
@@ -1084,13 +1148,17 @@
         if dlam is not None:
             dlam = dlam.to(lam_dtype).reshape(())
         wb = pack.weight
-        dx = None
-        if ctx.needs_input_grad[0]:
+        dx = dys = None
+        if ctx.needs_input_grad[0] or ctx.needs_input_grad[1]:
             if deep256_usable(M, wb.shape[1], wb.shape[0]):
                 dx = deep256(dy, pack, True, None).view(B, N, K)
             else:
                 dx = (_hip.linear_bf16(dy, pack.transposed(), None) if own_gemm(M, wb.shape[1], wb.shape[0]) else dy @ wb).view(B, N, K)
-        return (dx, None, None, None, None, None, None, dv0, dlam, None, None, None, None, *_pack_weight_grads(dy, x2.contiguous(), pack), *ograds)
+        if ctx.pro is not None:
+            xnew, y, mean, rstd = ln
+            dx, dys = ctx.pro.backward(xnew, y, mean, rstd, dx, dxnew, ctx.needs_input_grad[0])
+        return (dx, dys, None, None, None, None, None, None, None, None, dv0, dlam, None, None, None, None,
+                *_pack_weight_grads(dy, x2.contiguous(), pack), *ograds)
 
 
 def attention_core_usable(x: Tensor, pack: "PackedWeight", heads: int, d: int, wq: Tensor, wk: Tensor, cos: Tensor) -> bool:
@@ -1103,10 +1171,11 @@
 
 def attention_core(x: Tensor, pack: "PackedWeight", cos: Tensor, sin: Tensor, wq: Tensor, wk: Tensor, v0: Optional[Tensor],
                    lam: Optional[Tensor], heads: int, eps: float, scale: float, v0link: Optional[GradLink],
-                   out_pack: Optional["PackedWeight"] = None):
+                   out_pack: Optional["PackedWeight"] = None, prologue: Optional[LnPrologue] = None):
     oparams = () if out_pack is None else tuple(out_pack.params)
-    return _AttentionCore.apply(x, pack, out_pack, cos.contiguous(), sin.contiguous(), wq.contiguous(), wk.contiguous(), v0,
-                                lam if v0 is not None else None, heads, eps, scale, v0link, *pack.params, *oparams)
+    y, allm = (prologue.y, prologue.mods.allm) if prologue is not None else (None, None)
+    return _AttentionCore.apply(x, y, allm, prologue, pack, out_pack, cos.contiguous(), sin.contiguous(), wq.contiguous(), wk.contiguous(),
+                                v0, lam if v0 is not None else None, heads, eps, scale, v0link, *pack.params, *oparams)
 
 
 def row_pack(weights: list[Tensor], biases: Optional[list[Tensor]], pad_to: Optional[int] = None) -> PackedWeight:
diff --git a/viforsdes_amd/primitives/mlp.py b/viforsdes_amd/primitives/mlp.py
--- a/viforsdes_amd/primitives/mlp.py
+++ b/viforsdes_amd/primitives/mlp.py
@@ -1,4 +1,6 @@
 from __future__ import annotations
+
+from typing import Optional
 
 import torch
 from torch import Tensor, nn
@@ -37,7 +39,14 @@
             object.__setattr__(self, "_packs", packs)
         return packs
 
-    def forward(self, x: Tensor) -> Tensor:
+    def forward(self, x: Tensor, prologue: Optional["fused.LnPrologue"] = None):
+        if prologue is not None:
+            if (fused.ENABLED and fused.ln_prologue_usable(x) and fused.packed_linear_usable(x, 2 * self.padded_width(), self.in_dim)
+                    and fused.swiglu_mlp_usable(x, self.padded_width())):
+                packs = self.packs(x, True)
+                return fused.swiglu_mlp(x, packs[0], packs[1], prologue)
+            xnew, h = prologue.materialise()
+            return self.forward(h), xnew
         if fused.ENABLED and x.is_cuda and x.dtype in (torch.float32, torch.bfloat16) and not fused.fp16_autocast():
             width = self.padded_width()
             if fused.packed_linear_usable(x, 2 * width, self.in_dim):
diff --git a/viforsdes_amd/primitives/sit.py b/viforsdes_amd/primitives/sit.py
--- a/viforsdes_amd/primitives/sit.py
+++ b/viforsdes_amd/primitives/sit.py
@@ -115,11 +115,18 @@
             h1 = fused.ln_modulate_m(tokens, mods, (0, SA), (0, HA), blocks[0].attn_norm.eps, final=True, link=link0)
         v0: Optional[Tensor] = None
         v0link = fused.GradLink() if self.config.attn_residual_v else None
+        prologue = mods is not None and isinstance(blocks[0].mlp, SwiGLU) and fused.ln_prologue_usable(tokens)
+        pending: Optional[fused.LnPrologue] = None
         for k, blk in enumerate(blocks):
             block_form = (isinstance(blk.mlp, SwiGLU) and blk.mlp.input_proj.bias is not None
                           and fused.mlp_block_nograd_usable(tokens, mods, blk.mlp.padded_width())
                           and fused.swiglu_mlp_usable(tokens, blk.mlp.padded_width()))
-            attn_out, values = blk.self_attn.forward_fused(h1, rotary=rotary, v0=v0, v0link=v0link, defer_out=block_form)
+            if pending is not None:
+                attn_out, values, tokens = blk.self_attn.forward_fused(pending.x, rotary=rotary, v0=v0, v0link=v0link,
+                                                                       defer_out=block_form, prologue=pending)
+                pending = None
+            else:
+                attn_out, values = blk.self_attn.forward_fused(h1, rotary=rotary, v0=v0, v0link=v0link, defer_out=block_form)
             if v0 is None and self.config.attn_residual_v:
                 v0 = values
             lk = link0 if k == 0 else None
@@ -128,14 +135,19 @@
                 tokens, h1 = fused.mlp_block_nograd(tokens, attn_out, mods, k, k + 1 if k + 1 < nb else None, blk.mlp_norm.eps,
                                                     blocks[k + 1].attn_norm.eps if k + 1 < nb else blk.mlp_norm.eps, pin, pout)
                 continue
-            if mods is None:
-                x1, h2 = fused.residual_norm(tokens, attn_out, ml[k][GA], ml[k][SM], ml[k][HM], blk.mlp_norm.eps, lk)
+            if prologue:
+                mlp_out, x1 = blk.mlp(tokens, fused.LnPrologue(tokens, attn_out, mods, (k, GA), (k, SM), (k, HM), blk.mlp_norm.eps, lk))
             else:
-                x1, h2 = fused.residual_norm_m(tokens, attn_out, mods, (k, GA), (k, SM), (k, HM), blk.mlp_norm.eps, lk)
-            mlp_out = blk.mlp(h2)
+                if mods is None:
+                    x1, h2 = fused.residual_norm(tokens, attn_out, ml[k][GA], ml[k][SM], ml[k][HM], blk.mlp_norm.eps, lk)
+                else:
+                    x1, h2 = fused.residual_norm_m(tokens, attn_out, mods, (k, GA), (k, SM), (k, HM), blk.mlp_norm.eps, lk)
+                mlp_out = blk.mlp(h2)
             if k + 1 < nb:
                 eps = blocks[k + 1].attn_norm.eps
-                if mods is None:
+                if prologue:
+                    pending = fused.LnPrologue(x1, mlp_out, mods, (k, GM), (k + 1, SA), (k + 1, HA), eps)
+                elif mods is None:
                     tokens, h1 = fused.residual_norm(x1, mlp_out, ml[k][GM], ml[k + 1][SA], ml[k + 1][HA], eps)
                 else:
                     tokens, h1 = fused.residual_norm_m(x1, mlp_out, mods, (k, GM), (k + 1, SA), (k + 1, HA), eps)
```

After: 19780, median of 6. About the same (+0.1%).
